# abeytheo/gan-inpainting

Measured on AMD Instinct MI355X. Metric: training images/sec at 256x256 bs=32/GPU, higher is better.
Workload: dtype f16; 1 GPU; wgan_rmse 256x256 bs=32/GPU (BASELINE.json configs[3]): U-Net G (41.8M) + PatchGAN critic, RMSprop 5e-5, clip 0.01, RMSE recon, G update every 5th batch, random-init weights; global_batch=32, parallelism=dp1, compute=fp16 MFMA, fp32 accumulate, fp32 master weights

## Files before the change

### gan-inpainting_amd/backend.py

```python
import ctypes as C
import os
import threading

import torch

_HERE = os.path.dirname(os.path.abspath(__file__))
LIB_PATH = os.environ.get("GI_LIB_PATH") or os.path.join(_HERE, "libganinpaint.so")

GI_F32, GI_F16 = 0, 1
ACT_NONE, ACT_RELU, ACT_LRELU = 0, 1, 2

_vp, _i, _i64, _f, _u64 = C.c_void_p, C.c_int, C.c_int64, C.c_float, C.c_uint64

PROTOTYPES = {
    "gi_last_error": (C.c_char_p, []),
    "gi_version": (_i, []),
    "gi_set_option": (_i, [C.c_char_p, _i]),
    "gi_get_option": (_i, [C.c_char_p, C.POINTER(_i)]),
    "gi_debug_last_kernel": (C.c_char_p, []),
    "gi_debug_fold_count": (_i, []),
    "gi_ctx_create": (_i, [_i, _vp, C.POINTER(_vp)]),
    "gi_ctx_destroy": (_i, [_vp]),
    "gi_ctx_sync": (_i, [_vp]),
    "gi_unet_create": (_i, [_vp, _i, _i, _f, _i, _i, _i, _i, _i, C.POINTER(_vp)]),
    "gi_unet_create_ex": (_i, [_vp, _i, _i, _i, _f, _i, _i, _i, _i, _i, C.POINTER(_vp)]),
    "gi_unet_create_norm": (_i, [_vp, _i, _i, _i, _i, _f, _i, _i, _i, _i, _i, C.POINTER(_vp)]),
    "gi_unet_create_padded": (_i, [_vp, _i, _i, _i, _i, _i, _f, _i, _i, _i, _i, _i, C.POINTER(_vp)]),
    "gi_patchgan_create": (_i, [_vp, _i, _i, _i, _i, _i, _i, C.POINTER(_vp)]),
    "gi_patchgan_create_sn": (_i, [_vp, _i, _i, _i, _i, _i, _i, _i, _i, C.POINTER(_vp)]),
    "gi_net_sn_read": (_i, [_vp, _i, _vp, _vp, _i64]),
    "gi_dcgan_create": (_i, [_vp, _i, _i, _i, _i, _i, C.POINTER(_vp)]),
    "gi_dcgan_debug_forward_convs": (_i, [_vp, _i, _vp, _i]),
    "gi_net_destroy": (_i, [_vp]),
    "gi_net_tensor_count": (_i, [_vp]),
    "gi_net_tensor_desc": (_i, [_vp, _i, C.c_char_p, _i, C.POINTER(_i), C.POINTER(_i64), C.POINTER(_i),
                                C.POINTER(_i64), C.POINTER(_i64)]),
    "gi_net_param_floats": (_i64, [_vp]),
    "gi_net_buffer_floats": (_i64, [_vp]),
    "gi_net_workspace_bytes": (_i64, [_vp]),
    "gi_net_bind": (_i, [_vp, _vp, _vp, _vp, _vp, _i64]),
    "gi_net_sync_weights": (_i, [_vp]),
    "gi_net_set_train": (_i, [_vp, _i]),
    "gi_net_set_inference": (_i, [_vp, _i]),
    "gi_net_set_loss_scale": (_i, [_vp, _f]),
    "gi_net_set_bn_groups": (_i, [_vp, _i]),
    "gi_net_set_dropout_seed": (_i, [_vp, _u64]),
    "gi_net_get_dropout_state": (_i, [_vp, C.POINTER(_u64), C.POINTER(_u64)]),
    "gi_net_set_dropout_state": (_i, [_vp, _u64, _u64]),
    "gi_net_dropout_mask": (_i, [_vp, _i, _i, _vp, _i64]),
    "gi_net_saved_activation": (_i, [_vp, _i, _i, _i, _vp, _i64]),
    "gi_net_debug_nonzero_tickets": (_i, [_vp, _vp]),
    "gi_net_set_dropout_mask": (_i, [_vp, _i, _i, _vp]),
    "gi_net_forward": (_i, [_vp, _i, _vp, _vp, _i]),
    "gi_net_backward": (_i, [_vp, _i, _vp, _vp, _i]),
    "gi_net_backward_phase": (_i, [_vp, _i, _vp, _vp, _i, _i]),
    "gi_net_phase_split": (_i64, [_vp]),
    "gi_net_phase_split2": (_i64, [_vp]),
    "gi_comm_unique_id": (_i, [C.c_char_p]),
    "gi_comm_create": (_i, [C.c_char_p, _i, _i, _i, C.POINTER(_vp)]),
    "gi_comm_destroy": (_i, [_vp]),
    "gi_allreduce_sum_f32": (_i, [_vp, _vp, _i64, _vp]),
    "gi_net_allreduce_grads_async": (_i, [_vp, _vp, _i64, _i64, _vp]),
    "gi_allreduce_wait": (_i, [_vp, _vp, _vp]),
    "gi_patchgan_gradient_penalty": (_i, [_vp, _vp, _i, _f, _vp]),
    "gi_patchgan_gp_saved_activation": (_i, [_vp, _i, _vp, _i64]),
    "gi_interpolate": (_i, [_vp, _vp, _vp, _vp, _i, _i64, _vp]),
    "gi_mask_apply": (_i, [_vp, _vp, _vp, _vp, _vp, _i64, _i]),
    "gi_mask_composite": (_i, [_vp, _vp, _vp, _vp, _vp, _i64]),
    "gi_mul": (_i, [_vp, _vp, _vp, _vp, _i64]),
    "gi_add": (_i, [_vp, _vp, _vp, _vp, _i64, _f]),
    "gi_loss_l1": (_i, [_vp, _vp, _vp, _i64, _vp, _vp, _f, _vp]),
    "gi_loss_rmse": (_i, [_vp, _vp, _vp, _i64, _f, _vp, _vp, _f, _vp]),
    "gi_loss_mse": (_i, [_vp, _vp, _vp, _i64, _vp, _vp, _f, _vp]),
    "gi_loss_local": (_i, [_vp, _vp, _vp, _vp, _i64, _i, _vp, _vp, _f, _vp]),
    "gi_loss_adv": (_i, [_vp, _vp, _i, _i, _f, _vp, _vp, _f]),
    "gi_loss_adv_pair": (_i, [_vp, _vp, _i, _i, _f, _f, _vp, _vp, _vp, _f, _f]),
    "gi_adam_step": (_i, [_vp, _vp, _vp, _vp, _vp, _i64, _f, _f, _f, _f, _i, _f]),
    "gi_rmsprop_step": (_i, [_vp, _vp, _vp, _vp, _i64, _f, _f, _f, _f, _f]),
    "gi_clamp": (_i, [_vp, _vp, _i64, _f, _f]),
    "gi_grad_absmean": (_i, [_vp, _vp, _vp, _vp, _i, _vp]),
    "gi_ssim_scratch_floats": (_i64, [_i, _i, _i, _i, _i]),
    "gi_ssim": (_i, [_vp, _vp, _vp, _i, _i, _i, _i, _i, _vp, _vp, _vp, _vp]),
    "gi_eval_recon_scratch_floats": (_i64, [_i64]),
    "gi_eval_recon": (_i, [_vp, _vp, _vp, _vp, _i64, _f, _vp, _vp, _vp, _vp]),
    "gi_seg_metrics": (_i, [_vp, _vp, _vp, _i, _i, _i64, _vp, _i, _vp, _vp, _vp]),
    "gi_loss_tv": (_i, [_vp, _vp, _i, _i, _i, _f, _vp, _vp, _f, _vp]),
    "gi_loss_cross_entropy": (_i, [_vp, _vp, _vp, _i, _i, _i64, _vp, _i, _vp, _vp, _f, _vp]),
    "gi_vgg19_create": (_i, [_vp, _i, _i, _i, _vp]),
    "gi_vgg19_destroy": (None, [_vp]),
    "gi_vgg19_param_floats": (_i64, [_vp]),
    "gi_vgg19_workspace_bytes": (_i64, [_vp]),
    "gi_vgg19_num_tensors": (_i, [_vp]),
    "gi_vgg19_tensor_desc": (_i, [_vp, _i, _vp, _i, _vp, _vp]),
    "gi_vgg19_bind": (_i, [_vp, _vp, _vp, _i64]),
    "gi_vgg19_sync_weights": (_i, [_vp]),
    "gi_vgg19_perceptual_style": (_i, [_vp, _vp, _vp, _i, _f, _f, _vp, _vp]),
    "gi_vgg19_features": (_i, [_vp, _vp, _i, _i, _vp]),
    "gi_vgg19_grad_workspace_bytes": (_i64, [_vp]),
    "gi_vgg19_bind_grad": (_i, [_vp, _vp, _i64]),
    "gi_vgg19_perceptual_style_grad": (_i, [_vp, _vp, _vp, _i, _f, _f, _vp, _vp, _vp, _f]),
    "gi_vgg19_grad_layer": (_i, [_vp, _i, _vp]),
    "gi_lpips_create": (_i, [_vp, _i, _i, _i, _vp]),
    "gi_lpips_destroy": (None, [_vp]),
# ... 9 lines not shown
    "gi_lpips_bind_grad": (_i, [_vp, _vp, _i64]),
    "gi_lpips_distance_grad": (_i, [_vp, _vp, _vp, _i, _vp, _vp, _vp, _f]),
    "gi_lpips_grad_tap": (_i, [_vp, _i, _vp]),
    "gi_debug_lpips_pack_t": (_i, [_vp, _vp, _vp, _i, _i]),
    "gi_debug_lpips_seed": (_i, [_vp, _i, _vp, _i, _i, _i, _vp, _vp, _vp]),
    "gi_debug_lpips_scale": (_i, [_vp, _vp, _vp, _i]),
    "gi_debug_lpips_act_bwd": (_i, [_vp, _i, _vp, _vp, _vp, _vp, _i, _i, _i, _i, _i]),
    "gi_debug_lpips_conv1_adjoint": (_i, [_vp, _vp, _vp, _vp, _f, _vp, _i, _i, _i]),
    "gi_debug_lpips_conv1": (_i, [_vp, _vp, _vp, _i, _i, _i, _vp, _vp, _vp, _vp]),
    "gi_debug_lpips_fold": (_i, [_vp, _vp, _vp, _vp, _vp, _vp]),
    "gi_debug_lpips_tap_ws_bytes": (_i64, [_i]),
    "gi_debug_lpips_tap": (_i, [_vp, _vp, _i, _i, _i, _i, _vp, _vp, _i64, _vp, _vp]),
    "gi_inception_create": (_i, [_vp, _i, _i, _vp]),
    "gi_inception_destroy": (None, [_vp]),
    "gi_inception_param_floats": (_i64, [_vp]),
    "gi_inception_workspace_bytes": (_i64, [_vp]),
    "gi_inception_num_tensors": (_i, [_vp]),
    "gi_inception_tensor_desc": (_i, [_vp, _i, _vp, _i, _vp, _vp]),
    "gi_inception_bind": (_i, [_vp, _vp, _vp, _i64]),
    "gi_inception_sync_weights": (_i, [_vp]),
    "gi_inception_features": (_i, [_vp, _vp, _i, _i, _i, _i, _vp]),
    "gi_inception_debug_forward_convs": (_i, [_vp, _vp, _i, _i, _i, _i, _i]),
    "gi_inception_num_steps": (_i, [_vp]),
    "gi_inception_step_desc": (_i, [_vp, _i, _vp, _vp, _vp, _vp, _vp]),
    "gi_inception_debug_forward_steps": (_i, [_vp, _vp, _i, _i, _i, _i, _i]),
    "gi_inception_debug_read": (_i, [_vp, _i, _i, _i, _vp]),
    "gi_fid_stats_acc_doubles": (_i64, [_i]),
    "gi_fid_stats_update": (_i, [_vp, _vp, _vp, _i, _i]),
    "gi_fid_stats_finish": (_i, [_vp, _vp, _vp, _vp, _i]),
    "gi_featmetrics_workspace_bytes": (_i64, [_i, _i64, _i64, _i]),
    "gi_kid_subset_sums": (_i, [_vp, _vp, _vp, _vp, _vp, _i, _i, _i, _vp, _i64, _vp]),
    "gi_feat_knn_radius": (_i, [_vp, _vp, _i, _i, _i, _vp, _i64, _vp]),
    "gi_feat_manifold_members": (_i, [_vp, _vp, _i, _vp, _vp, _i, _i, _vp, _i64, _vp, _vp]),
    "gi_debug_feat_gram": (_i, [_vp, _vp, _vp, _i, _vp, _vp, _i, _i, _vp]),
    "gi_resize_output_size": (_i, [_i, _i, _i, _vp, _vp]),
    "gi_resize_table_bytes": (_i64, [_i, _i, _i, _i]),
    "gi_resize_build_tables": (_i, [_vp, _i, _i, _i, _i, _vp]),
    "gi_resize_to_tensor": (_i, [_vp, _vp, _vp, _i, _i, _i, _i, _i, _vp, _vp, _vp]),
    "gi_mask_generate": (_i, [_vp, _i, _u64, _vp, _i, _i, _i, _vp, _vp]),
    "gi_batch_gather": (_i, [_vp, _vp, _i64, _i, _i, _vp, _i, _vp, _u64, _i, _vp]),
    "gi_image_quantize": (_i, [_vp, _vp, _i64, _vp]),
    "gi_panel_assemble": (_i, [_vp, _vp, _i, _i, _i, _i, _i, _vp]),
    "gi_mask_bbox": (_i, [_vp, _vp, _i, _i, _i, _vp]),
    "gi_window_crop": (_i, [_vp, _vp, _i, _i, _i, _i, _i, _i, _i, _vp]),
    "gi_feather_paste": (_i, [_vp, _vp, _vp, _i, _i, _i, _i, _i, _i, _vp, _i, _vp]),
    "gi_mask_components_workspace_bytes": (C.c_size_t, [_i, _i, _i]),
    "gi_mask_components": (_i, [_vp, _vp, _i, _i, _i, _i, _vp, _vp, _vp, _vp]),
    "gi_diffaug_params": (_i, [_vp, _i, _u64, _u64, _i, _i, _i, _vp]),
    "gi_diffaug_fwd": (_i, [_vp, _vp, _vp, _i, _i, _i, _i, _vp]),
    "gi_diffaug_bwd": (_i, [_vp, _vp, _vp, _i, _i, _i, _i, _vp]),
    "gi_diffaug_apply": (_i, [_vp, _i, _u64, _u64, _vp, _i, _i, _i, _vp]),
    "gi_diffaug_apply_bwd": (_i, [_vp, _i, _u64, _u64, _vp, _i, _i, _i, _vp]),
    "gi_check_finite": (_i, [_vp, _vp, _i64, _vp]),
    "gi_check_finite_scan": (_i, [_vp, _vp, _i64, _vp]),
    "gi_check_finite_finish": (_i, [_vp, _vp]),
    "gi_adam_step_guarded": (_i, [_vp, _vp, _vp, _vp, _vp, _i64, _f, _f, _f, _f, _i, _f, _vp]),
    "gi_adam_step_guarded2": (_i, [_vp, _vp, _vp, _vp, _vp, _i64, _f, _f, _f, _f, _i, _i, _f, _vp]),
    "gi_rmsprop_step_guarded": (_i, [_vp, _vp, _vp, _vp, _i64, _f, _f, _f, _f, _f, _vp]),
    "gi_check_finite_scan_word": (_i, [_vp, _vp, _i64, _vp, _i]),
    "gi_adam_step_scan": (_i, [_vp, _vp, _vp, _vp, _vp, _i64, _f, _f, _f, _f, _i, _i, _f, _vp, _i, _i]),
    "gi_rmsprop_step_scan": (_i, [_vp, _vp, _vp, _vp, _i64, _f, _f, _f, _f, _f, _vp, _i, _i]),
    "gi_ema_update": (_i, [_vp, _vp, _vp, _i64, _f, _vp]),
    "gi_wgrad_s2_scratch_bytes": (_i64, [_i, _i, _i, _i, _i, _i]),
    "gi_wgrad_s2_ws": (_i, [_vp, _i, _vp, _vp, _vp, _i, _i, _i, _i, _i, _i, _i, _i, _f, _vp, _i64]),
    "gi_c1_gather": (_i, [_vp, _i, _vp, _vp, _vp, _i, _i, _i, _i, _i, _i, _i, _f, _vp, _vp, _vp]),
    "gi_c1_scatter": (_i, [_vp, _i, _vp, _vp, _vp, _vp, _i, _i, _i, _i, _i, _i, _i, _i, _f, _vp, _vp, _vp, _i, _vp, _vp]),
    "gi_c1_wgrad": (_i, [_vp, _i, _vp, _vp, _vp, _i, _i, _i, _i, _i, _i, _i, _f, _f, _vp, _i, _vp, _vp, _vp, _i64]),
    "gi_c1_wgrad_reduce": (_i, [_vp, _vp, _vp, _i, _i, _vp, _i64]),
    "gi_c1_head4_col_bytes": (_i64, [_i, _i, _i]),
    "gi_c1_head4_forward": (_i, [_vp, _vp, _vp, _vp, _vp, _vp, _i, _i, _i, _i, _i, _i, _vp]),
    "gi_c1_head4_dgrad": (_i, [_vp, _vp, _vp, _vp, _i, _i, _i, _i, _i]),
    "gi_conv_s2_forward": (_i, [_vp, _i, _vp, _vp, _vp, _i, _i, _i, _i, _i, _i, _i, _i, _i, _vp, _i64]),
    "gi_convT_s2_forward": (_i, [_vp, _i, _vp, _vp, _vp, _i, _i, _i, _i, _i, _i, _i, _i, _i, _vp, _i64]),
    "gi_wgrad_s2": (_i, [_vp, _i, _vp, _vp, _vp, _i, _i, _i, _i, _i, _i, _i, _i, _f]),
    "gi_conv_s2_forward_ex": (_i, [_vp, _i, _vp, _vp, _vp, _i, _i, _i, _i, _i, _i, _i, _i, _i, _vp, _i64, _vp]),
    "gi_convT_s2_forward_ex": (_i, [_vp, _i, _vp, _vp, _vp, _i, _i, _i, _i, _i, _i, _i, _i, _i, _vp, _i64, _vp]),
    "gi_debug_igemm_plan": (_i, [_i, _i, _i, _i, _i, _i, _i, _i, _i, _i, _i, _i64, _i, _vp, _i, _vp]),
    "gi_stat_acc_words": (_i64, [_i]),
    "gi_stat_acc_read": (_i, [_vp, _vp, _i, _i, _i, _vp]),
    "gi_debug_col_stats": (_i, [_vp, _i, _vp, _i64, _i, _vp, C.POINTER(_i)]),
    "gi_debug_bn_finalize": (_i, [_vp, _vp, _i, _i, _i64, _vp, _vp, _vp, _vp, _vp, _vp, _vp, _vp, _i, _f, _f, _i, _i64, _i]),
    "gi_debug_bn_apply": (_i, [_vp, _i, _vp, _vp, _i64, _i, _i, _i, _vp, _vp, _i, _vp, _f, _i64, _i]),
    "gi_debug_bn_finalize_acc": (_i, [_vp, _i, _vp]),
    "gi_debug_bn_apply_acc": (_i, [_vp, _i, _vp, _vp, _i64, _i, _i, _i, _i, _vp, _f, _u64, _f, _vp, _vp, _vp, _i64]),
    "gi_debug_act_bn_bwd": (_i, [_vp, _i, _vp]),
    "gi_debug_in_forward": (_i, [_vp, _i, _vp, _vp, _i, _i, _i, _i, _i, _i, _vp, _f, _f, _vp]),
    "gi_debug_act_in_bwd": (_i, [_vp, _i, _vp, _i, _i, _vp]),
    "gi_debug_bias_grad": (_i, [_vp, _i, _vp, _i64, _i, _f, _vp, _vp]),
    "gi_debug_tanh_bwd": (_i, [_vp, _vp, _vp, _vp, _i64, _f]),
    "gi_debug_fill_dropout": (_i, [_vp, _vp, _i64, _u64, _f]),
    "gi_debug_mask_layout": (_i, [_vp, _vp, _vp, _i, _i, _i, _i]),
    "gi_debug_mul_slope": (_i, [_vp, _i, _vp, _vp, _vp, _i64]),
    "gi_debug_bn_tangent_inject": (_i, [_vp, _i, _vp, _vp, _vp, _vp, _vp, _i64, _i, _vp, _vp, _vp, _vp, _f, _vp, _vp]),
    "gi_debug_gp_direction": (_i, [_vp, _vp, _i, _i64, _f, _vp, _vp, _vp, _vp, _vp]),
    "gi_debug_gp_unscale_add": (_i, [_vp, _vp, _vp, _vp, _i64]),
    "gi_debug_sn_power_iteration": (_i, [_vp, _vp, _i, _i, _i, _vp, _vp, _i, _i, _vp]),
    "gi_debug_sn_project_add": (_i, [_vp, _vp, _vp, _vp, _vp, _vp, _i, _i, _i, _vp, _vp]),
    "gi_debug_stat_acc_add": (_i, [_vp, _vp, _i, _i, _i, _i, _vp, _i]),
    "gi_debug_pack_weights_batch": (_i, [_vp, _i, _vp, _i]),
    "gi_debug_head_forward": (_i, [_vp, _i, _vp]),
    "gi_debug_head_backward": (_i, [_vp, _i, _vp]),
    "gi_debug_head_scratch_bytes": (_i64, [_i, _i, _i]),
    "gi_debug_vgg_conv3x3": (_i, [_vp, _vp, _vp, _vp, _vp, _i, _i, _i, _i, _i, _i, _vp, _i, _i, _vp, _vp, C.POINTER(_i), C.POINTER(_i)]),
    "gi_debug_vgg_conv1": (_i, [_vp, _vp, _vp, _i, _i, _i, _vp, _vp, _vp, _vp]),
    "gi_debug_vgg_maxpool2": (_i, [_vp, _vp, _vp, _i, _i, _i, _i]),
    "gi_debug_vgg_tap_ws_bytes": (_i64, []),
    "gi_debug_vgg_tap_terms": (_i, [_vp, _vp, _i, _i, _i, _i, _vp, _i64, _vp, _vp, _vp, C.POINTER(_i)]),
    "gi_debug_vgg_seed": (_i, [_vp, _i, _vp, _vp, _vp, _vp, _vp, _vp, _i, _i, _i, _f, _f]),
    "gi_debug_vgg_scale": (_i, [_vp, _vp, _vp]),
    "gi_debug_vgg_act_bwd": (_i, [_vp, _i, _vp, _vp, _vp, _vp, _i, _i, _i, _i, _i]),
    "gi_debug_vgg_conv1_adjoint": (_i, [_vp, _vp, _vp, _vp, _f, _vp, _i, _i, _i]),
    "gi_pack_weights": (_i, [_vp, _i, _vp, _i, _i, _vp, _vp]),
    "gi_convert": (_i, [_vp, _i, _vp, _vp, _i64]),
    "gi_convert_back": (_i, [_vp, _i, _vp, _vp, _i64]),
    "gi_time_convT_s2": (_i, [_vp, _i, _vp, _vp, _vp, _i, _i, _i, _i, _i, _i, _i, _i, C.POINTER(_f)]),
    "gi_time_conv_s2": (_i, [_vp, _i, _vp, _vp, _vp, _i, _i, _i, _i, _i, _i, _i, _i, C.POINTER(_f)]),
}

_lib = None
_lock = threading.Lock()


class IgemmEx(C.Structure):
    _fields_ = [("relu_cend", _i),
                ("mask", _vp), ("ldmask", _i), ("mask_slope", _f),
                ("add", _vp), ("ldadd", _i),
                ("mask_bits", _vp),
                ("stat_acc", _vp), ("stat_reps", _i), ("stat_pg", _i),
                ("partials", _vp),
                ("bwd_x", _vp), ("bwd_ldx", _i),
                ("bwd_scale", _vp), ("bwd_shift", _vp), ("bwd_mean", _vp), ("bwd_inv", _vp), ("bwd_stride", _i),
                ("bwd_slope", _f), ("bwd_acc", _vp), ("bwd_reps", _i), ("bwd_pg", _i64),
                ("bwd_c0", _i), ("bwd_c", _i),
                ("mask_applied", _i), ("bwd_applied", _i), ("stat_used", _i), ("ntiles_out", _i)]


class BnAccArgs(C.Structure):
    _fields_ = [("acc", _vp), ("reps", _i),
                ("gamma", _vp), ("beta", _vp), ("running_mean", _vp), ("running_var", _vp),
                ("scale", _vp), ("shift", _vp), ("save_mean", _vp), ("save_invstd", _vp),
                ("count", _i64), ("momentum", _f), ("eps", _f), ("groups", _i), ("out_stride", _i),
                ("zero_next", _vp), ("zero_words", _i)]


class ActBnBwdArgs(C.Structure):
    _fields_ = [("g1", _vp), ("ldg1", _i), ("coffg1", _i),
                ("g2", _vp), ("ldg2", _i), ("coffg2", _i),
                ("y", _vp), ("ldy", _i), ("coffy", _i),
                ("x", _vp), ("dx", _vp),
                ("pixels", _i64), ("c", _i), ("act", _i), ("drop_scale", _f),
                ("has_bn", _i), ("eval_bn", _i),
                ("gamma", _vp), ("save_mean", _vp), ("save_invstd", _vp),
                ("dgamma", _vp), ("dbeta", _vp), ("inv_loss_scale", _f),
                ("partials", _vp), ("sums", _vp), ("fwd_scale", _vp), ("fwd_shift", _vp),
                ("groups", _i), ("stat_stride", _i),
                ("acc", _vp), ("acc_reps", _i), ("zero_next", _vp), ("zero_words", _i),
                ("reduce_done", _i)]


class PackJob(C.Structure):
    _fields_ = [("w", _vp), ("packed", _vp), ("phase", _vp),
                ("ca", _i), ("cb", _i), ("scale_on_b", _i),
                ("scale", _vp)]


class HeadArgs(C.Structure):
# ... 98 lines not shown
```

### gan-inpainting_amd/csrc/api.hip

```cpp
#include <string.h>

#include <stdlib.h>

#include "common.h"
#include "stat_acc.h"
#include "igemm_plan.h"

static thread_local char g_err[1024] = "";

void gi_set_error(const char* fmt, ...) {
  va_list ap;
  va_start(ap, fmt);
  vsnprintf(g_err, sizeof(g_err), fmt, ap);
  va_end(ap);
}

namespace {
struct OptDesc { const char* name; int dflt; int value; int state; };
inline int opt_load(const int& v) { return __atomic_load_n(&v, __ATOMIC_RELAXED); }
inline void opt_store(int& v, int x) { __atomic_store_n(&v, x, __ATOMIC_RELAXED); }
OptDesc g_opts[GI_OPT_COUNT] = {
  {"GI_IGEMM5", 7, 0, 0}, {"GI_IGEMM6", 1, 0, 0}, {"GI_IGEMM7", 1, 0, 0}, {"GI_IGEMM_FIXUP", 1, 0, 0}, {"GI_IGEMM_VARIANT", 3, 0, 0},
  {"GI_BN_ACC", 1, 0, 0}, {"GI_FUSE_HEAD", 1, 0, 0}, {"GI_HEAD_FAST", 1, 0, 0}, {"GI_BN_BWD_FUSE", 1, 0, 0}, {"GI_BN_BWD_SMALL", 512, 0, 0},
  {"GI_WGRAD2", 1, 0, 0}, {"GI_WGRAD3", 1, 0, 0}, {"GI_IGEMM8", 1, 0, 0}, {"GI_BN_FOLD", 0, 0, 0}, {"GI_C1_FUSED", 1, 0, 0},
  {"GI_WGRAD_STREAM", 1, 0, 0}, {"GI_MASK_BITS", 1, 0, 0}, {"GI_C1W_FUSE", 1, 0, 0}, {"GI_IGEMM7_WAVES", 8, 0, 0},
};
thread_local const char* g_last_kernel = "";
int g_fold_count = 0;
}
void gi_note_fold() { __atomic_fetch_add(&g_fold_count, 1, __ATOMIC_RELAXED); }

int gi_opt(int id) {
  OptDesc& o = g_opts[id];
  if (opt_load(o.state) == 0) {
    const char* e = getenv(o.name);
    opt_store(o.value, e ? atoi(e) : o.dflt);
    __atomic_store_n(&o.state, 1, __ATOMIC_RELEASE);
  }
  return opt_load(o.value);
}
void gi_note_kernel(const char* name) { g_last_kernel = name; }

extern "C" {

int gi_set_option(const char* name, int value) {
  GI_REQUIRE(name, "set_option: null name");
  for (int i = 0; i < GI_OPT_COUNT; ++i)
    if (strcmp(name, g_opts[i].name) == 0) {
      if (value < 0) opt_store(g_opts[i].state, 0);
      else { opt_store(g_opts[i].value, value); __atomic_store_n(&g_opts[i].state, 2, __ATOMIC_RELEASE); }
      return GI_OK;
    }
  gi_set_error("set_option: unknown option '%s'", name);
  return GI_ERR_INVALID;
}
int gi_get_option(const char* name, int* value) {
  GI_REQUIRE(name && value, "get_option: null argument");
  for (int i = 0; i < GI_OPT_COUNT; ++i)
    if (strcmp(name, g_opts[i].name) == 0) { *value = gi_opt(i); return GI_OK; }
  gi_set_error("get_option: unknown option '%s'", name);
  return GI_ERR_INVALID;
}
const char* gi_debug_last_kernel(void) { return g_last_kernel; }
int gi_debug_fold_count(void) { return __atomic_load_n(&g_fold_count, __ATOMIC_RELAXED); }

const char* gi_last_error(void) { return g_err; }
int gi_version(void) { return 100; }

int gi_ctx_create(int device_id, void* hip_stream, gi_ctx** out) {
  GI_REQUIRE(out != nullptr, "ctx_create: out is null");
  int count = 0;
  GI_HIP(hipGetDeviceCount(&count));
  GI_REQUIRE(device_id >= 0 && device_id < count, "ctx_create: device %d not present (%d visible)", device_id, count);
  GI_HIP(hipSetDevice(device_id));
  hipDeviceProp_t prop;
  GI_HIP(hipGetDeviceProperties(&prop, device_id));
  if (strncmp(prop.gcnArchName, "gfx950", 6) != 0) {
    gi_set_error("ctx_create: device %d is %s; this library is built for gfx950 only", device_id, prop.gcnArchName);
    return GI_ERR_UNSUPPORTED;
  }
  gi_ctx* c = new gi_ctx();
  c->device = device_id;
  c->stream = (hipStream_t)hip_stream;
  *out = c;
  return GI_OK;
}
int gi_ctx_destroy(gi_ctx* ctx) {
  if (ctx && ctx->tickets) (void)hipFree(ctx->tickets);
  if (ctx && ctx->absmean_partials) (void)hipFree(ctx->absmean_partials);
  if (ctx && ctx->diffaug_partials) (void)hipFree(ctx->diffaug_partials);
  delete ctx;
  return GI_OK;
}
int gi_ctx_sync(gi_ctx* ctx) {
  GI_REQUIRE(ctx, "ctx_sync: null");
  GI_HIP(hipStreamSynchronize(ctx->stream));
  return GI_OK;
}

static unsigned* ctx_tickets(gi_ctx* ctx) {
  if (!ctx->tickets) {
    if (hipMalloc((void**)&ctx->tickets, GI_IGEMM_TICKETS * 4) != hipSuccess) { ctx->tickets = nullptr; return nullptr; }
    if (hipMemset(ctx->tickets, 0, GI_IGEMM_TICKETS * 4) != hipSuccess) { (void)hipFree(ctx->tickets); ctx->tickets = nullptr; }
  }
  return ctx->tickets;
}

int gi_conv_s2_forward(gi_ctx* ctx, int dtype, const void* in, const void* w_packed, void* out, int n, int H, int W, int cb, int ldin,
                       int ca, int ldout, int relu_in, int act_out, float* ws, int64_t ws_bytes) {
  GI_REQUIRE(ctx && in && w_packed && out, "conv_s2_forward: null pointer");
  GI_REQUIRE(H % 2 == 0 && W % 2 == 0, "conv_s2_forward: H=%d W=%d must be even", H, W);
  IgemmArgs a;
  memset(&a, 0, sizeof(a));
  a.in = in; a.w = w_packed; a.out = out; a.ws = ws; a.ws_bytes = ws_bytes;
  a.tickets = ws ? ctx_tickets(ctx) : nullptr;
  a.n = n; a.Hs = H / 2; a.Ws = W / 2;
  a.cin = cb; a.ldin = ldin; a.cout = ca; a.ldout = ldout;
  a.relu_in = relu_in; a.act_out = act_out;
  return op_igemm(ctx->stream, dtype, 0, a);
}

int gi_convT_s2_forward(gi_ctx* ctx, int dtype, const void* in, const void* w_phase, void* out, int n, int H, int W, int ca, int ldin,
                        int cb, int ldout, int relu_in, int act_out, float* ws, int64_t ws_bytes) {
  GI_REQUIRE(ctx && in && w_phase && out, "convT_s2_forward: null pointer");
  IgemmArgs a;
  memset(&a, 0, sizeof(a));
  a.in = in; a.w = w_phase; a.out = out; a.ws = ws; a.ws_bytes = ws_bytes;
  a.tickets = ws ? ctx_tickets(ctx) : nullptr;
  a.n = n; a.Hs = H; a.Ws = W;
  a.cin = ca; a.ldin = ldin; a.cout = cb; a.ldout = ldout;
  a.relu_in = relu_in; a.act_out = act_out;
  return op_igemm(ctx->stream, dtype, 1, a);
}

static int apply_ex(IgemmArgs& a, const gi_igemm_ex* ex) {
  if (!ex) return GI_OK;
  GI_REQUIRE(ex->relu_cend >= 0 && ex->relu_cend % 64 == 0 && ex->relu_cend <= a.cin, "igemm_ex: relu_cend=%d must be a multiple of 64 within the %d input channels",
             ex->relu_cend, a.cin);
  a.relu_cend = ex->relu_cend;
  a.mask = ex->mask; a.ldmask = ex->ldmask; a.mask_slope = ex->mask_slope;
  a.add = ex->add; a.ldadd = ex->ldadd;
  a.mask_bits = ex->mask ? ex->mask_bits : nullptr;
  a.stat_acc = ex->stat_acc; a.stat_reps = ex->stat_reps; a.stat_pg = ex->stat_pg;
  a.partials = ex->partials;
  a.bwd_x = ex->bwd_x; a.bwd_ldx = ex->bwd_ldx; a.bwd_scale = ex->bwd_scale; a.bwd_shift = ex->bwd_shift; a.bwd_mean = ex->bwd_mean;
  a.bwd_inv = ex->bwd_inv; a.bwd_stride = ex->bwd_stride; a.bwd_slope = ex->bwd_slope; a.bwd_acc = ex->bwd_acc; a.bwd_reps = ex->bwd_reps;
  a.bwd_pg = ex->bwd_pg;
  a.bwd_c0 = ex->bwd_c0; a.bwd_c = ex->bwd_c;
  return GI_OK;
}
static void return_ex(const IgemmArgs& a, gi_igemm_ex* ex) {
  if (!ex) return;
  ex->mask_applied = a.mask_applied; ex->bwd_applied = a.bwd_applied; ex->stat_used = a.stat_used; ex->ntiles_out = a.ntiles_out;
}

int gi_conv_s2_forward_ex(gi_ctx* ctx, int dtype, const void* in, const void* w_packed, void* out, int n, int H, int W, int cb, int ldin,
                          int ca, int ldout, int relu_in, int act_out, float* ws, int64_t ws_bytes, gi_igemm_ex* ex) {
  GI_REQUIRE(ctx && in && w_packed && out, "conv_s2_forward_ex: null pointer");
  GI_REQUIRE(H % 2 == 0 && W % 2 == 0, "conv_s2_forward_ex: H=%d W=%d must be even", H, W);
  IgemmArgs a;
  memset(&a, 0, sizeof(a));
  a.in = in; a.w = w_packed; a.out = out; a.ws = ws; a.ws_bytes = ws_bytes;
  a.tickets = ws ? ctx_tickets(ctx) : nullptr;
  a.n = n; a.Hs = H / 2; a.Ws = W / 2;
  a.cin = cb; a.ldin = ldin; a.cout = ca; a.ldout = ldout;
  a.relu_in = relu_in; a.act_out = act_out;
  GI_TRY(apply_ex(a, ex));
  const int rc = op_igemm(ctx->stream, dtype, 0, a);
  return_ex(a, ex);
  return rc;
}

int gi_convT_s2_forward_ex(gi_ctx* ctx, int dtype, const void* in, const void* w_phase, void* out, int n, int H, int W, int ca, int ldin,
                           int cb, int ldout, int relu_in, int act_out, float* ws, int64_t ws_bytes, gi_igemm_ex* ex) {
  GI_REQUIRE(ctx && in && w_phase && out, "convT_s2_forward_ex: null pointer");
  IgemmArgs a;
  memset(&a, 0, sizeof(a));
  a.in = in; a.w = w_phase; a.out = out; a.ws = ws; a.ws_bytes = ws_bytes;
  a.tickets = ws ? ctx_tickets(ctx) : nullptr;
  a.n = n; a.Hs = H; a.Ws = W;
  a.cin = ca; a.ldin = ldin; a.cout = cb; a.ldout = ldout;
  a.relu_in = relu_in; a.act_out = act_out;
  GI_TRY(apply_ex(a, ex));
  const int rc = op_igemm(ctx->stream, dtype, 1, a);
  return_ex(a, ex);
  return rc;
}

int gi_debug_igemm_plan(int dtype, int mode, int n, int Hs, int Ws, int cin, int ldin, int cout, int ldout, int relu_in, int act_out,
                        int64_t ws_bytes, int has_tickets, const gi_igemm_ex* ex, int offered, gi_igemm_plan_info* out) {
  GI_REQUIRE(out, "debug_igemm_plan: null pointer");
  static char dummy[8];
  IgemmArgs a;
  memset(&a, 0, sizeof(a));
  a.in = a.w = a.out = dummy;
  if (ws_bytes > 0) { a.ws = (float*)dummy; a.ws_bytes = ws_bytes; }
  a.tickets = has_tickets ? (unsigned*)dummy : nullptr;
  a.n = n; a.Hs = Hs; a.Ws = Ws;
  a.cin = cin; a.ldin = ldin; a.cout = cout; a.ldout = ldout;
  a.relu_in = relu_in; a.act_out = act_out;
  GI_TRY(apply_ex(a, ex));
  IgemmFold fold = {};
  if ((offered & 1) && a.stat_acc) { fold.bn.groups = 1; fold.bn.acc = a.stat_acc; fold.lddst = ldout; fold.act = GI_ACT_RELU; a.fold = &fold; }
  if ((offered & 2) && a.mask_bits) { a.c1w_img = (const float*)dummy; a.c1w_part = (float*)dummy; a.c1w_part_floats = (int64_t)1 << 40; a.c1w_scale = 1.f; }
  if (offered & 4) a.pool2 = 1;
  if (offered & 8) a.bias = (const float*)dummy;
  IgemmPlan p;
  GI_TRY(gi_igemm_plan(dtype, mode, a, &p));
  gi_igemm_returns(p, a);
  memset(out, 0, sizeof(*out));
  strncpy(out->name, p.name, sizeof(out->name) - 1);
  out->grid = p.grid; out->splitk = p.splitk > 1 ? p.splitk : 1; out->ntiles_out = a.ntiles_out;
  out->mask_applied = a.mask_applied; out->bwd_applied = a.bwd_applied; out->stat_used = a.stat_used;
  out->c1w_applied = a.c1w_applied; out->c1w_blocks = a.c1w_blocks; out->pool_applied = a.pool_applied; out->fold_applied = a.fold_applied;
  return GI_OK;
}

int64_t gi_stat_acc_words(int c) { return gi_stat_block_words(c, GI_STAT_MAXREP); }

namespace {
__global__ void __launch_bounds__(256) stat_acc_read_kernel(const unsigned long long* acc, int c, int reps, int group, double* out) {
  for (int ch = blockIdx.x * 256 + threadIdx.x; ch < c; ch += gridDim.x * 256) {
    out[ch] = gi_stat_read(acc, c, reps, group, 0, ch);
    out[c + ch] = gi_stat_read(acc, c, reps, group, 1, ch);
  }
}
}

int gi_stat_acc_read(gi_ctx* ctx, const unsigned long long* acc, int c, int reps, int group, double* out_dev) {
  GI_REQUIRE(ctx && acc && out_dev && c > 0 && reps >= 1 && reps <= GI_STAT_MAXREP && (group == 0 || group == 1), "stat_acc_read: bad argument");
  hipLaunchKernelGGL(stat_acc_read_kernel, dim3((c + 255) / 256), dim3(256), 0, ctx->stream, acc, c, reps, group, out_dev);
  GI_LAUNCH_CHECK();
  return GI_OK;
}

int gi_wgrad_s2(gi_ctx* ctx, int dtype, const void* S, const void* L, float* dW, int n, int Hs, int Ws, int ca, int ldS, int cb, int ldL,
                int relu_S, float scale) {
  GI_REQUIRE(ctx && S && L && dW, "wgrad_s2: null pointer");
  WgradArgs a;
  a.S = S; a.L = L; a.dW = dW; a.n = n; a.Hs = Hs; a.Ws = Ws;
  a.ca = ca; a.ldS = ldS; a.coffS = 0; a.cb = cb; a.ldL = ldL; a.coffL = 0;
  a.relu_S = relu_S; a.scale = scale;
  a.scratch = nullptr; a.scratch_bytes = 0;
  return op_wgrad(ctx->stream, dtype, a);
}

int64_t gi_wgrad_s2_scratch_bytes(int dtype, int n, int Hs, int Ws, int ca, int cb) {
  return op_wgrad_scratch_bytes(dtype, n, Hs, Ws, ca, cb);
}

int gi_wgrad_s2_ws(gi_ctx* ctx, int dtype, const void* S, const void* L, float* dW, int n, int Hs, int Ws, int ca, int ldS, int cb, int ldL,
                   int relu_S, float scale, float* scratch, int64_t scratch_bytes) {
  GI_REQUIRE(ctx && S && L && dW, "wgrad_s2_ws: null pointer");
  WgradArgs a;
  a.S = S; a.L = L; a.dW = dW; a.n = n; a.Hs = Hs; a.Ws = Ws;
  a.ca = ca; a.ldS = ldS; a.coffS = 0; a.cb = cb; a.ldL = ldL; a.coffL = 0;
  a.relu_S = relu_S; a.scale = scale;
  a.scratch = scratch; a.scratch_bytes = scratch_bytes;
  return op_wgrad(ctx->stream, dtype, a);
}


int gi_c1_gather(gi_ctx* ctx, int dtype, const float* img, const float* w, void* out, int n, int Hs, int Ws, int c, int ldout, int coffout,
                 int act_out, float in_scale, const float* bias, unsigned long long* bits, int* bits_written) {
  GI_REQUIRE(ctx && img && w && out, "c1_gather: null pointer");
  return op_c1_gather(ctx->stream, dtype, img, w, out, n, Hs, Ws, c, ldout, coffout, act_out, in_scale, bias, bits, bits_written);
}

int gi_c1_scatter(gi_ctx* ctx, int dtype, const void* X, const float* w, const float* bias, float* img, int n, int Hs, int Ws, int c, int ldx,
                  int coffx, int relu_in, int post, float out_scale, void* col_scratch, float* img2, const void* x2, int ld2,
                  const float* scale2, const float* shift2) {
  GI_REQUIRE(ctx && X && w && img, "c1_scatter: null pointer");
  GI_REQUIRE(!x2 || (scale2 && shift2), "c1_scatter: x2 without scale2 / shift2");
  C1Affine aff;
  aff.x2 = x2; aff.ld2 = ld2; aff.scale = scale2; aff.shift = shift2;
  return op_c1_scatter(ctx->stream, dtype, X, w, bias, img, n, Hs, Ws, c, ldx, coffx, relu_in, post, out_scale, col_scratch, img2,
                       x2 ? &aff : nullptr);
}

int gi_c1_wgrad(gi_ctx* ctx, int dtype, const void* X, const float* img, float* dW, int n, int Hs, int Ws, int c, int ldx, int coffx,
                int relu_in, float scale, float img_scale, const void* x2, int ld2, const float* scale2, const float* shift2, float* scratch,
                int64_t scratch_floats) {
  GI_REQUIRE(ctx && X && img && dW, "c1_wgrad: null pointer");
  GI_REQUIRE(!x2 || (scale2 && shift2), "c1_wgrad: x2 without scale2 / shift2");
  C1Affine aff;
  aff.x2 = x2; aff.ld2 = ld2; aff.scale = scale2; aff.shift = shift2;
  return op_c1_wgrad(ctx->stream, dtype, X, img, dW, n, Hs, Ws, c, ldx, coffx, relu_in, scale, img_scale, x2 ? &aff : nullptr, scratch,
                     scratch_floats);
}
// ... 23 lines not shown
inline bool dbg_act_ok(int act) { return act == GI_ACT_NONE || act == GI_ACT_RELU || act == GI_ACT_LRELU; }
inline bool dbg_c_ok(int dtype, int c) { const int e = dbg_epc(dtype); return c > 0 && c % e == 0 && gi_is_pow2(c / e) && c / e <= 256; }
inline bool dbg_view_ok(int dtype, int c, int ld, int coff) { const int e = dbg_epc(dtype); return coff >= 0 && coff % e == 0 && ld % e == 0 && coff + c <= ld; }

int dbg_bn_acc(const char* who, int c, const gi_bn_acc_args* b, BnAccArgs& o) {
  GI_REQUIRE(b && b->acc && b->gamma && b->beta && b->running_mean && b->running_var && b->scale && b->shift && b->save_mean && b->save_invstd,
             "%s: null pointer", who);
  GI_REQUIRE(b->reps >= 1 && b->reps <= GI_STAT_MAXREP, "%s: reps=%d outside 1..%d", who, b->reps, GI_STAT_MAXREP);
  GI_REQUIRE(b->groups == 1 || b->groups == 2, "%s: groups=%d (1 or 2)", who, b->groups);
  GI_REQUIRE(b->count >= 1, "%s: count=%lld", who, (long long)b->count);
  GI_REQUIRE(b->groups == 1 || b->out_stride >= c, "%s: out_stride=%d below the %d channels", who, b->out_stride, c);
  GI_REQUIRE(b->zero_words >= 0 && (b->zero_words == 0 || b->zero_next), "%s: zero_words=%d without zero_next", who, b->zero_words);
  o.acc = b->acc; o.reps = b->reps; o.gamma = b->gamma; o.beta = b->beta; o.running_mean = b->running_mean; o.running_var = b->running_var;
  o.scale = b->scale; o.shift = b->shift; o.save_mean = b->save_mean; o.save_invstd = b->save_invstd;
  o.count = b->count; o.momentum = b->momentum; o.eps = b->eps; o.groups = b->groups; o.out_stride = b->out_stride;
  o.zero_next = b->zero_words > 0 ? b->zero_next : nullptr; o.zero_words = b->zero_words;
  return GI_OK;
}

int dbg_bwd_args(const char* who, int dtype, const gi_act_bn_bwd_args* s, bool chunks_pow2, ActBnBwdArgs& a) {
  GI_REQUIRE(s && s->dx, "%s: null pointer", who);
  GI_REQUIRE(dbg_dtype_ok(dtype) && dbg_act_ok(s->act), "%s: dtype=%d act=%d", who, dtype, s->act);
  GI_REQUIRE(chunks_pow2 ? dbg_c_ok(dtype, s->c) : (s->c > 0 && s->c % dbg_epc(dtype) == 0), "%s: c=%d unsupported", who, s->c);
  GI_REQUIRE(s->pixels >= 1, "%s: pixels=%lld", who, (long long)s->pixels);
  GI_REQUIRE(s->g1 || s->g2, "%s: no upstream gradient", who);
  GI_REQUIRE(!s->g1 || dbg_view_ok(dtype, s->c, s->ldg1, s->coffg1), "%s: g1 ld=%d coff=%d for %d channels", who, s->ldg1, s->coffg1, s->c);
  GI_REQUIRE(!s->g2 || dbg_view_ok(dtype, s->c, s->ldg2, s->coffg2), "%s: g2 ld=%d coff=%d for %d channels", who, s->ldg2, s->coffg2, s->c);
  GI_REQUIRE(!s->y || dbg_view_ok(dtype, s->c, s->ldy, s->coffy), "%s: y ld=%d coff=%d for %d channels", who, s->ldy, s->coffy, s->c);
  GI_REQUIRE(s->drop_scale == 1.f || s->act == GI_ACT_RELU,
             "%s: drop_scale=%g with act=%d: the backward takes the dropout zeros from y > 0, which only a ReLU output can carry", who,
             (double)s->drop_scale, s->act);
  memset(&a, 0, sizeof(a));
  a.g1 = s->g1; a.ldg1 = s->ldg1; a.coffg1 = s->coffg1;
  a.g2 = s->g2; a.ldg2 = s->ldg2; a.coffg2 = s->coffg2;
  a.y = s->y; a.ldy = s->ldy; a.coffy = s->coffy;
  a.x = s->x; a.dx = s->dx; a.pixels = s->pixels; a.c = s->c; a.act = s->act; a.drop_scale = s->drop_scale;
  a.has_bn = s->has_bn; a.eval_bn = s->eval_bn;
  a.gamma = s->gamma; a.save_mean = s->save_mean; a.save_invstd = s->save_invstd;
  a.dgamma = s->dgamma; a.dbeta = s->dbeta; a.inv_loss_scale = s->inv_loss_scale;
  a.partials = s->partials; a.sums = s->sums; a.fwd_scale = s->fwd_scale; a.fwd_shift = s->fwd_shift;
  a.groups = s->groups; a.stat_stride = s->stat_stride;
  a.acc = s->acc; a.acc_reps = s->acc_reps; a.zero_next = s->zero_words > 0 ? s->zero_next : nullptr; a.zero_words = s->zero_words;
  a.reduce_done = s->reduce_done;
  return GI_OK;
}

__global__ void __launch_bounds__(256) stat_acc_add_kernel(unsigned long long* acc, int c, int reps, int group, int q, const float* addends) {
  const int r = blockIdx.x;
  for (int ch = threadIdx.x; ch < c; ch += 256) gi_stat_add(acc, c, r & (reps - 1), group, q, ch, addends[(int64_t)r * c + ch]);
}
}

int gi_debug_col_stats(gi_ctx* ctx, int dtype, const void* x, int64_t pixels, int c, float* partials, int* rows_out) {
  GI_REQUIRE(ctx && x && partials && rows_out, "debug_col_stats: null pointer");
  GI_REQUIRE(dbg_dtype_ok(dtype) && pixels >= 1, "debug_col_stats: dtype=%d pixels=%lld", dtype, (long long)pixels);
  return op_col_stats(ctx->stream, dtype, x, pixels, c, partials, rows_out);
}

int gi_debug_bn_finalize(gi_ctx* ctx, const float* partials, int rows, int c, int64_t count, const float* gamma, const float* beta,
                         float* running_mean, float* running_var, float* scale, float* shift, float* save_mean, float* save_invstd, int train,
                         float momentum, float eps, int groups, int64_t part_stride, int out_stride) {
  GI_REQUIRE(ctx && gamma && beta && running_mean && running_var && scale && shift && save_mean && save_invstd, "debug_bn_finalize: null pointer");
  GI_REQUIRE(!train || (partials && rows >= 1), "debug_bn_finalize: train mode needs partial rows (rows=%d)", rows);
  GI_REQUIRE(c >= 1 && count >= 1, "debug_bn_finalize: c=%d count=%lld", c, (long long)count);
  GI_REQUIRE(groups == 1 || groups == 2, "debug_bn_finalize: groups=%d (1 or 2)", groups);
  GI_REQUIRE(groups == 1 || (out_stride >= c && (!train || part_stride >= (int64_t)rows * 2 * c)),
             "debug_bn_finalize: two populations overlap (part_stride=%lld out_stride=%d)", (long long)part_stride, out_stride);
  return op_bn_finalize(ctx->stream, partials, rows, c, count, gamma, beta, running_mean, running_var, scale, shift, save_mean, save_invstd, train,
                        momentum, eps, groups, part_stride, out_stride);
}

int gi_debug_bn_apply(gi_ctx* ctx, int dtype, const void* x, void* y, int64_t pixels, int c, int ldy, int coffy, const float* scale,
                      const float* shift, int act, const uint8_t* drop_mask, float drop_scale, int64_t pg, int gstride) {
  GI_REQUIRE(ctx && x && y, "debug_bn_apply: null pointer");
  GI_REQUIRE(dbg_dtype_ok(dtype) && dbg_act_ok(act) && pixels >= 1, "debug_bn_apply: dtype=%d act=%d pixels=%lld", dtype, act, (long long)pixels);
  GI_REQUIRE(dbg_c_ok(dtype, c), "debug_bn_apply: c=%d unsupported", c);
  GI_REQUIRE(dbg_view_ok(dtype, c, ldy, coffy), "debug_bn_apply: ldy=%d coffy=%d for %d channels", ldy, coffy, c);
  GI_REQUIRE((scale == nullptr) == (shift == nullptr), "debug_bn_apply: scale and shift go together");
  GI_REQUIRE(pg >= 0 && pg <= pixels, "debug_bn_apply: pg=%lld of %lld pixels", (long long)pg, (long long)pixels);
  GI_REQUIRE(!(pg > 0 && pg < pixels) || gstride >= c, "debug_bn_apply: gstride=%d below the %d channels", gstride, c);
  return op_bn_apply(ctx->stream, dtype, x, y, pixels, c, ldy, coffy, scale, shift, act, drop_mask, drop_scale, pg, gstride);
}

int gi_debug_bn_finalize_acc(gi_ctx* ctx, int c, const gi_bn_acc_args* b) {
  GI_REQUIRE(ctx && c >= 1, "debug_bn_finalize_acc: bad argument");
  BnAccArgs o;
  GI_TRY(dbg_bn_acc("debug_bn_finalize_acc", c, b, o));
  return op_bn_finalize_acc(ctx->stream, c, o);
}

int gi_debug_bn_apply_acc(gi_ctx* ctx, int dtype, const void* x, void* y, int64_t pixels, int c, int ldy, int coffy, int act, uint8_t* drop_mask,
                          float drop_scale, uint64_t drop_seed, float drop_p, const gi_bn_acc_args* b, const void* side_src, void* side_dst,
                          int64_t side_bytes) {
  GI_REQUIRE(ctx && x && y, "debug_bn_apply_acc: null pointer");
  GI_REQUIRE(dbg_dtype_ok(dtype) && dbg_act_ok(act) && pixels >= 1, "debug_bn_apply_acc: dtype=%d act=%d pixels=%lld", dtype, act, (long long)pixels);
  GI_REQUIRE(dbg_c_ok(dtype, c), "debug_bn_apply_acc: c=%d unsupported", c);
  GI_REQUIRE(dbg_view_ok(dtype, c, ldy, coffy), "debug_bn_apply_acc: ldy=%d coffy=%d for %d channels", ldy, coffy, c);
  GI_REQUIRE(drop_p >= 0.f && drop_p < 1.f && (drop_p == 0.f || drop_mask), "debug_bn_apply_acc: drop_p=%g needs a mask to store the draw", (double)drop_p);
  GI_REQUIRE(side_bytes >= 0, "debug_bn_apply_acc: side_bytes=%lld", (long long)side_bytes);
  BnAccArgs o;
  GI_TRY(dbg_bn_acc("debug_bn_apply_acc", c, b, o));
  return op_bn_apply_acc(ctx->stream, dtype, x, y, pixels, c, ldy, coffy, act, drop_mask, drop_scale, drop_seed, drop_p, o, side_src, side_dst,
                         side_bytes);
}

int gi_debug_act_bn_bwd(gi_ctx* ctx, int dtype, const gi_act_bn_bwd_args* s) {
  GI_REQUIRE(ctx, "debug_act_bn_bwd: null context");
  ActBnBwdArgs a;
  GI_TRY(dbg_bwd_args("debug_act_bn_bwd", dtype, s, true, a));
  GI_REQUIRE(a.groups == 1 || a.groups == 2, "debug_act_bn_bwd: groups=%d (1 or 2)", a.groups);
  GI_REQUIRE(a.groups == 1 || a.stat_stride >= a.c, "debug_act_bn_bwd: stat_stride=%d below the %d channels", a.stat_stride, a.c);
  GI_REQUIRE(!a.has_bn || (a.x && a.gamma && a.save_mean && a.save_invstd), "debug_act_bn_bwd: BatchNorm without x / gamma / save_mean / save_invstd");
  GI_REQUIRE((a.fwd_scale == nullptr) == (a.fwd_shift == nullptr), "debug_act_bn_bwd: fwd_scale and fwd_shift go together");
  const bool need_y = a.g2 != nullptr || a.act != GI_ACT_NONE;
  GI_REQUIRE(!need_y || a.y || (a.has_bn && a.fwd_scale), "debug_act_bn_bwd: the activation's sign needs y or fwd_scale / fwd_shift");
  GI_REQUIRE(!a.acc || (a.acc_reps >= 1 && a.acc_reps <= GI_STAT_MAXREP), "debug_act_bn_bwd: acc_reps=%d outside 1..%d", a.acc_reps, GI_STAT_MAXREP);
  GI_REQUIRE(!a.reduce_done || (a.acc && a.has_bn && !a.eval_bn), "debug_act_bn_bwd: reduce_done needs train-mode accumulators");
  GI_REQUIRE(!a.has_bn || a.acc || (a.partials && a.sums), "debug_act_bn_bwd: BatchNorm without accumulators needs partials and sums");
  GI_REQUIRE(a.zero_words >= 0, "debug_act_bn_bwd: zero_words=%d", a.zero_words);
  return op_act_bn_bwd(ctx->stream, dtype, a);
}

int gi_debug_in_forward(gi_ctx* ctx, int dtype, const void* x, void* y, int n, int hw, int c, int ldy, int coffy, int act,
                        const uint8_t* drop_mask, float drop_scale, float eps, float* stats) {
  GI_REQUIRE(ctx && x && y && stats, "debug_in_forward: null pointer");
  GI_REQUIRE(dbg_dtype_ok(dtype) && dbg_act_ok(act), "debug_in_forward: dtype=%d act=%d", dtype, act);
  GI_REQUIRE(c > 0 && c % dbg_epc(dtype) == 0 && dbg_view_ok(dtype, c, ldy, coffy), "debug_in_forward: c=%d ldy=%d coffy=%d", c, ldy, coffy);
  return op_in_forward(ctx->stream, dtype, x, y, n, hw, c, ldy, coffy, act, drop_mask, drop_scale, eps, stats);
}

int gi_debug_act_in_bwd(gi_ctx* ctx, int dtype, const gi_act_bn_bwd_args* s, int n, int hw, const float* stats) {
  GI_REQUIRE(ctx && stats, "debug_act_in_bwd: null pointer");
  ActBnBwdArgs a;
  GI_TRY(dbg_bwd_args("debug_act_in_bwd", dtype, s, false, a));
  GI_REQUIRE(n >= 1 && hw >= 1, "debug_act_in_bwd: n=%d hw=%d", n, hw);
  const bool need_y = a.g2 != nullptr || a.act != GI_ACT_NONE;
  GI_REQUIRE(!need_y || a.y, "debug_act_in_bwd: the activation's sign needs y");
  return op_act_in_bwd(ctx->stream, dtype, a, n, hw, stats);
}

int gi_debug_bias_grad(gi_ctx* ctx, int dtype, const void* dz, int64_t pixels, int c, float scale, float* dbias, float* partials) {
  GI_REQUIRE(ctx && dz && dbias && partials, "debug_bias_grad: null pointer");
  GI_REQUIRE(dbg_dtype_ok(dtype) && pixels >= 1, "debug_bias_grad: dtype=%d pixels=%lld", dtype, (long long)pixels);
  return op_bias_grad(ctx->stream, dtype, dz, pixels, c, scale, dbias, partials);
}

int gi_debug_tanh_bwd(gi_ctx* ctx, const float* dy, const float* y, float* dx, int64_t count, float scale) {
  GI_REQUIRE(ctx && dy && y && dx && count >= 0, "debug_tanh_bwd: bad argument");
  return op_tanh_bwd(ctx->stream, dy, y, dx, count, scale);
}

int gi_debug_fill_dropout(gi_ctx* ctx, uint8_t* mask_nhwc, int64_t count, uint64_t seed, float p) {
  GI_REQUIRE(ctx && mask_nhwc && count >= 0, "debug_fill_dropout: bad argument");
  GI_REQUIRE(p >= 0.f && p < 1.f, "debug_fill_dropout: p=%g outside [0, 1)", (double)p);
  return op_fill_dropout(ctx->stream, mask_nhwc, count, seed, p);
}

int gi_debug_mask_layout(gi_ctx* ctx, const uint8_t* src, uint8_t* dst, int n, int c, int hw, int to_nhwc) {
  GI_REQUIRE(ctx && src && dst && src != dst, "debug_mask_layout: bad pointer");
  GI_REQUIRE(n >= 1 && c >= 1 && hw >= 1, "debug_mask_layout: n=%d c=%d hw=%d", n, c, hw);
  return op_mask_nchw_to_nhwc(ctx->stream, src, dst, n, c, hw, to_nhwc);
}

int gi_debug_mul_slope(gi_ctx* ctx, int dtype, const void* tin, const void* a, void* tout, int64_t count) {
  GI_REQUIRE(ctx && tin && a && tout, "debug_mul_slope: null pointer");
  GI_REQUIRE(dbg_dtype_ok(dtype) && count >= 0, "debug_mul_slope: dtype=%d count=%lld", dtype, (long long)count);
// ... 178 lines not shown
```

### gan-inpainting_amd/csrc/bn_acc.h

```cpp
#pragma once
#include "common.h"
#include "stat_acc.h"

struct BnAccP {
  const unsigned long long* acc;
  int reps;
  const float* gamma; const float* beta;
  float* rmean; float* rvar;
  float* scale; float* shift; float* smean; float* sinv;
  double count;
  float momentum, eps;
  int groups, out_stride;
  unsigned long long* zero_next;
  int zero_words;
};
static inline void gi_fill_acc_params(BnAccP& fa, const BnAccArgs& b) {
  fa.acc = b.acc; fa.reps = b.reps > 0 ? b.reps : 1; fa.gamma = b.gamma; fa.beta = b.beta; fa.rmean = b.running_mean; fa.rvar = b.running_var;
  fa.scale = b.scale; fa.shift = b.shift; fa.smean = b.save_mean; fa.sinv = b.save_invstd;
  fa.count = (double)b.count; fa.momentum = b.momentum; fa.eps = b.eps; fa.groups = b.groups; fa.out_stride = b.out_stride;
  fa.zero_next = b.zero_next; fa.zero_words = b.zero_words;
}
__device__ __forceinline__ void zero_words64(unsigned long long* p, int n) {
  for (int i = threadIdx.x; i < n; i += 256) p[i] = 0ull;
}
template <bool COHERENT = false>
__device__ __forceinline__ void bn_from_acc(const BnAccP& a, int c, int ch, int j, bool write, float& sc_out, float& sh_out) {
  const float gam = a.gamma[ch], bet = a.beta[ch];
  float rm = 0.f, rv = 0.f;
  if (write) { rm = a.rmean[ch]; rv = a.rvar[ch]; }
  double t0, t1;
  gi_stat_read2<COHERENT>(a.acc, c, a.reps, j, ch, t0, t1);
  const double m = t0 / a.count;
  double v = t1 / a.count - m * m;
  if (v < 0.0 || a.count <= 1.0) v = 0.0;
  const float mean = (float)m, var = (float)v;
  const float inv = 1.0f / sqrtf(var + a.eps);
  const float sc = gam * inv;
  sc_out = sc;
  sh_out = bet - mean * sc;
  if (write) {
    const float unbiased = a.count > 1.0 ? (float)(v * a.count / (a.count - 1.0)) : var;
    a.rmean[ch] = (1.f - a.momentum) * rm + a.momentum * mean;
    a.rvar[ch] = (1.f - a.momentum) * rv + a.momentum * unbiased;
    const int o = j * a.out_stride + ch;
    a.scale[o] = sc;
    a.shift[o] = sh_out;
    a.smean[o] = mean;
    a.sinv[o] = inv;
  }
}

__host__ __device__ __forceinline__ uint64_t gi_mix64(uint64_t z) {
  z = (z ^ (z >> 30)) * 0xBF58476D1CE4E5B9ull;
  z = (z ^ (z >> 27)) * 0x94D049BB133111EBull;
  return z ^ (z >> 31);
}
constexpr uint64_t GI_GOLDEN64 = 0x9E3779B97F4A7C15ull;
__device__ __forceinline__ uint8_t dropout_keep(uint64_t seed, int64_t i, uint32_t thresh) {
  const uint64_t z = gi_mix64(seed + GI_GOLDEN64 * (uint64_t)(i + 1));
  return ((uint32_t)(z >> 32) >= thresh) ? 1 : 0;
}
static inline uint32_t gi_dropout_thresh(float p) {
  const double t = (double)p * 4294967296.0;
  const uint32_t thresh = t >= 4294967295.0 ? 0xFFFFFFFFu : (uint32_t)t;
  return thresh ? thresh : 1u;
}
```

### gan-inpainting_amd/csrc/common.h

```cpp
#pragma once
#include <hip/hip_runtime.h>
#include <stdint.h>
#include <stdio.h>
#include <stdarg.h>
#include <mutex>
#include <type_traits>

#include "../../include/ganinpaint.h"

typedef _Float16 half_t;
typedef _Float16 h8_t __attribute__((ext_vector_type(8)));
typedef _Float16 h4_t __attribute__((ext_vector_type(4)));
typedef _Float16 h2_t __attribute__((ext_vector_type(2)));
typedef __fp16 fp16x4_t __attribute__((__vector_size__(4 * sizeof(__fp16))));
typedef float f4_t __attribute__((ext_vector_type(4)));
typedef unsigned int u4_t __attribute__((ext_vector_type(4)));
typedef float f16_t __attribute__((ext_vector_type(16)));

void gi_set_error(const char* fmt, ...);

enum gi_opt_id {
  GI_OPT_IGEMM5 = 0, GI_OPT_IGEMM6, GI_OPT_IGEMM7, GI_OPT_IGEMM_FIXUP, GI_OPT_IGEMM_VARIANT, GI_OPT_BN_ACC, GI_OPT_FUSE_HEAD,
  GI_OPT_HEAD_FAST, GI_OPT_BN_BWD_FUSE, GI_OPT_BN_BWD_SMALL, GI_OPT_WGRAD2, GI_OPT_WGRAD3, GI_OPT_IGEMM8, GI_OPT_BN_FOLD, GI_OPT_C1_FUSED, GI_OPT_WGRAD_STREAM, GI_OPT_MASK_BITS, GI_OPT_C1W_FUSE, GI_OPT_IGEMM7_WAVES, GI_OPT_COUNT
};
int gi_opt(int id);
void gi_note_kernel(const char* name);
void gi_note_fold();
#ifdef GI_ABLATION
#include <stdlib.h>
static inline int gi_tune(const char* env, int dflt) { const char* e = getenv(env); return e ? atoi(e) : dflt; }
#else
#define gi_tune(env, dflt) (dflt)
#endif

template <int N, typename F>
__host__ __device__ __forceinline__ void static_for(F&& f) {
  if constexpr (N > 0) {
    static_for<N - 1>(f);
    f(std::integral_constant<int, N - 1>{});
  }
}

template <int ACT>
__device__ __forceinline__ float gi_act_c(float v) {
  if constexpr (ACT == GI_ACT_RELU) return v > 0.f ? v : 0.f;
  else if constexpr (ACT == GI_ACT_LRELU) return v > 0.f ? v : 0.2f * v;
  else return v;
}
template <typename F>
__device__ __forceinline__ void gi_with_act(int act, F&& f) {
  if (act == GI_ACT_NONE) f(std::integral_constant<int, GI_ACT_NONE>{});
  else if (act == GI_ACT_RELU) f(std::integral_constant<int, GI_ACT_RELU>{});
  else f(std::integral_constant<int, GI_ACT_LRELU>{});
}
template <typename F>
__host__ __device__ __forceinline__ void gi_with_bool(bool b, F&& f) {
  if (b) f(std::true_type{});
  else f(std::false_type{});
}
template <int CTRL>
__device__ __forceinline__ float gi_dpp(float v) {
  return __builtin_bit_cast(float, __builtin_amdgcn_update_dpp(0, __builtin_bit_cast(int, v), CTRL, 0xF, 0xF, true));
}
__device__ __forceinline__ float gi_row16_sum(float v) {
  v += gi_dpp<0xB1>(v);
  v += gi_dpp<0x4E>(v);
  v += gi_dpp<0x141>(v);
  v += gi_dpp<0x140>(v);
  return v;
}

__device__ __forceinline__ f4_t gi_ordered_sum_f4(const f4_t* part, int64_t stride, int k0, int k1, f4_t s) {
  int k = k0;
  for (; k + 8 <= k1; k += 8) {
    f4_t v[8];
#pragma unroll
    for (int j = 0; j < 8; ++j) v[j] = part[(int64_t)(k + j) * stride];
#pragma unroll
    for (int j = 0; j < 8; ++j) s += v[j];
  }
  if (k + 4 <= k1) {
    f4_t v[4];
#pragma unroll
    for (int j = 0; j < 4; ++j) v[j] = part[(int64_t)(k + j) * stride];
#pragma unroll
    for (int j = 0; j < 4; ++j) s += v[j];
    k += 4;
  }
  if (k + 2 <= k1) {
    const f4_t v0 = part[(int64_t)k * stride], v1 = part[(int64_t)(k + 1) * stride];
    s += v0;
    s += v1;
    k += 2;
  }
  if (k < k1) s += part[(int64_t)k * stride];
  return s;
}

struct GiDevOnce {
  unsigned long long mask = 0;
  std::mutex mu;
  bool first() {
    int d = 0;
    (void)hipGetDevice(&d);
    const unsigned long long b = 1ull << (d & 63);
    const unsigned long long old = __atomic_fetch_or(&mask, b, __ATOMIC_RELAXED);
    return (old & b) == 0;
  }
  template <typename F>
  hipError_t once(F&& f) {
    int d = 0;
    (void)hipGetDevice(&d);
    const unsigned long long b = 1ull << (d & 63);
    if (__atomic_load_n(&mask, __ATOMIC_ACQUIRE) & b) return hipSuccess;
    std::lock_guard<std::mutex> lock(mu);
    if (__atomic_load_n(&mask, __ATOMIC_RELAXED) & b) return hipSuccess;
    const hipError_t e = f();
    if (e == hipSuccess) __atomic_fetch_or(&mask, b, __ATOMIC_RELEASE);
    return e;
  }
};

#define GI_HIP(expr)                                                                  \
// ... 14 lines not shown
    }                                                                                 \
  } while (0)

#define GI_REQUIRE(cond, ...)                                                         \
  do {                                                                                \
    if (!(cond)) {                                                                    \
      gi_set_error(__VA_ARGS__);                                                      \
      return GI_ERR_INVALID;                                                          \
    }                                                                                 \
  } while (0)

#define GI_TRY(expr)                \
  do {                              \
    int _s = (expr);                \
    if (_s != GI_OK) return _s;     \
  } while (0)

template <auto Kernel, typename P>
int gi_launch_lds(dim3 grid, int block, int lds, int lds_attr, hipStream_t st, const P& p) {
  static GiDevOnce attr_set;
  GI_HIP(attr_set.once([&] { return hipFuncSetAttribute((const void*)Kernel, hipFuncAttributeMaxDynamicSharedMemorySize, lds_attr); }));
  hipLaunchKernelGGL(Kernel, grid, dim3(block), lds, st, p);
  GI_LAUNCH_CHECK();
  return GI_OK;
}

struct gi_ctx {
  int device;
  hipStream_t stream;
  unsigned* tickets = nullptr;
  double* absmean_partials = nullptr;
  double* diffaug_partials = nullptr;
};

static inline size_t gi_dtype_size(int dtype) { return dtype == GI_F16 ? 2 : 4; }
static inline int64_t gi_align_up(int64_t v, int64_t a) { return (v + a - 1) / a * a; }
static inline int gi_ilog2(int v) {
  int l = 0;
  while ((1 << l) < v) ++l;
  return l;
}
static inline bool gi_is_pow2(int v) { return v > 0 && (v & (v - 1)) == 0; }
static inline int grid_for(int64_t work_items, int per_block, int cap) {
  int64_t b = (work_items + per_block - 1) / per_block;
  if (b > cap) b = cap;
  if (b < 1) b = 1;
  return (int)b;
}


struct IgemmFold;
struct IgemmArgs {
  const void* in;
  const void* w;
  void* out;
  const float* bias;
  float* partials;
  float* ws;
  int64_t ws_bytes;
  int n, Hs, Ws;
  int cin, ldin, coffin;
  int cout, ldout, coffout;
  int relu_in;
  int relu_cend;
  int act_out;
  int force_splitk;
  unsigned* tickets;
  int ntiles_out;
  const void* mask; int ldmask, coffmask; float mask_slope;
  const void* add; int ldadd, coffadd;
  int mask_applied;
  const unsigned long long* mask_bits;
  const float* c1w_img; float* c1w_part; int64_t c1w_part_floats; float c1w_scale; int c1w_skip_out;
  int c1w_applied, c1w_blocks;
  unsigned long long* stat_acc; int stat_pg; int stat_reps;
  const void* bwd_x; int bwd_ldx;
  const float* bwd_scale; const float* bwd_shift; const float* bwd_mean; const float* bwd_inv; int bwd_stride;
  float bwd_slope; int bwd_c0, bwd_c;
  unsigned long long* bwd_acc; int bwd_reps; int64_t bwd_pg;
  int bwd_applied;
  int pool2, pool_applied;
  int stat_used;
  const IgemmFold* fold; int fold_applied;
};
constexpr int GI_IGEMM_TICKETS = 1024;
int op_igemm(hipStream_t st, int dtype, int mode, IgemmArgs& a);

struct WgradArgs {
  const void* S;
  const void* L;
  float* dW;
  int n, Hs, Ws;
  int ca, ldS, coffS;
  int cb, ldL, coffL;
  int relu_S;
  float scale;
  float* scratch;
  int64_t scratch_bytes;
};
int op_wgrad(hipStream_t st, int dtype, const WgradArgs& a);
int64_t op_wgrad_scratch_bytes(int dtype, int n, int Hs, int Ws, int ca, int cb);

int op_c1_gather(hipStream_t st, int dtype, const float* img, const float* w, void* out, int n, int Hs,
                 int Ws, int c, int ldout, int coffout, int act_out, float in_scale, const float* bias = nullptr,
                 unsigned long long* bits = nullptr, int* bits_written = nullptr);
struct BnAccArgs;
struct C1Affine { const void* x2; int ld2; const float* scale; const float* shift;
                  const BnAccArgs* bn = nullptr; };
bool op_c1_head4_ok(int dtype, int c, int out_c, int Ws, int ldx, int coffx);
int64_t op_c1_head4_col_bytes(int n, int Hs, int Ws);
int op_c1_head4_forward(hipStream_t st, const void* X, const float* w, const float* bias, float* out, float* out2, int n, int Hs, int Ws, int ldx,
                        int coffx, int relu_in, void* col_scratch);
int op_c1_head4_dgrad(hipStream_t st, const float* g, const float* w, void* out, int n, int Hs, int Ws, int ldout, int coffout);
int op_c1_wgrad_reduce(hipStream_t st, const float* part, float* dW, int count, int blocks, float* scratch = nullptr, int64_t scratch_floats = 0);
bool op_c1_affine_ok(int dtype, int c, int Ws, int ldx, int coffx);
int op_c1_scatter(hipStream_t st, int dtype, const void* X, const float* w, const float* bias, float* img,
                  int n, int Hs, int Ws, int c, int ldx, int coffx, int relu_in, int post, float out_scale,
                  void* col_scratch, float* img2 = nullptr, const C1Affine* aff = nullptr);
int op_c1_wgrad(hipStream_t st, int dtype, const void* X, const float* img, float* dW, int n, int Hs, int Ws,
                int c, int ldx, int coffx, int relu_in, float scale, float img_scale, const C1Affine* aff = nullptr,
                float* scratch = nullptr, int64_t scratch_floats = 0);

int op_bn_finalize(hipStream_t st, const float* partials, int rows, int c, int64_t count, const float* gamma,
                   const float* beta, float* running_mean, float* running_var, float* scale, float* shift,
                   float* save_mean, float* save_invstd, int train, float momentum, float eps, int groups = 1,
                   int64_t part_stride = 0, int out_stride = 0);
struct BnAccArgs {
  const unsigned long long* acc; int reps;
  const float* gamma; const float* beta;
  float* running_mean; float* running_var;
  float* scale; float* shift; float* save_mean; float* save_invstd;
  int64_t count;
  float momentum, eps;
  int groups, out_stride;
  unsigned long long* zero_next; int zero_words;
};
int op_bn_finalize_acc(hipStream_t st, int c, const BnAccArgs& b);
struct IgemmFold {
  BnAccArgs bn;
  void* dst; int lddst, coffdst;
  int act;
  uint8_t* drop_mask; float drop_scale; uint64_t drop_seed; float drop_p;
};
int op_bn_apply_acc(hipStream_t st, int dtype, const void* x, void* y, int64_t pixels, int c, int ldy, int coffy, int act,
                    uint8_t* drop_mask, float drop_scale, uint64_t drop_seed, float drop_p, const BnAccArgs& b,
                    const void* side_src = nullptr, void* side_dst = nullptr, int64_t side_bytes = 0);
int op_bn_apply(hipStream_t st, int dtype, const void* x, void* y, int64_t pixels, int c, int ldy, int coffy,
                const float* scale, const float* shift, int act, const uint8_t* drop_mask, float drop_scale,
                int64_t pg = 0, int gstride = 0);
int op_col_stats(hipStream_t st, int dtype, const void* x, int64_t pixels, int c, float* partials, int* rows_out);

struct ActBnBwdArgs {
  const void* g1; int ldg1, coffg1;
  const void* g2; int ldg2, coffg2;
  const void* y;  int ldy, coffy;
  const void* x;
  void* dx;
  int64_t pixels; int c;
  int act; float drop_scale;
  int has_bn;
  int eval_bn;
  const float* gamma; const float* save_mean; const float* save_invstd;
  float* dgamma; float* dbeta;
  float inv_loss_scale;
  float* partials;
  float* sums;
// ... 98 lines not shown
```

### gan-inpainting_amd/csrc/igemm7.hip

```cpp
#include <stdlib.h>

#include "common.h"
#include "stat_acc.h"
#include "bn_acc.h"
#include "igemm_plan.h"

namespace {

struct KP7 {
  const char* in;
  const char* w;
  char* out;
  const char* zero;
  const float* bias;
  float* partials;
  unsigned long long* stat_acc; int stat_pg, stat_reps;
  float* ws;
  unsigned* tickets;
  int M, Hs, Ws;
  int cin, ldin, coffin;
  int cout, ldout, coffout;
  int Ktot, nk, splitk, kt_per_split;
  int relu_in, act_out, relu_cend;
  int Hin, Win, Hout, Wout;
  int mtiles, ntiles;
  int dbg;
  int fold;
  unsigned* col_tickets;
  BnAccP fa;
  char* fdst; int flddst, fcoffdst, fact;
  uint8_t* fdrop; float fdrop_scale; uint64_t fdrop_seed; uint32_t fdrop_thresh;
};

__device__ __forceinline__ h8_t relu7(h8_t v, short floor) {
  typedef short s8_t __attribute__((ext_vector_type(8)));
  s8_t h = __builtin_bit_cast(s8_t, v);
  const s8_t z = {floor, floor, floor, floor, floor, floor, floor, floor};
  h = __builtin_elementwise_max(h, z);
  return __builtin_bit_cast(h8_t, h);
}
__device__ __forceinline__ void glds16_7(const char* src, char* lds_wave_base) {
  __builtin_amdgcn_global_load_lds((const __attribute__((address_space(1))) void*)src, (__attribute__((address_space(3))) void*)lds_wave_base,
                                   16, 0, 0);
}
template <int N>
__device__ __forceinline__ void wait_vm7() {
  static_assert(N >= 0 && N <= 63, "unexpected DMA count");
  if constexpr (N == 0) asm volatile("s_waitcnt vmcnt(0)" ::: "memory");
  else if constexpr (N == 3) asm volatile("s_waitcnt vmcnt(3)" ::: "memory");
  else if constexpr (N == 4) asm volatile("s_waitcnt vmcnt(4)" ::: "memory");
  else if constexpr (N == 6) asm volatile("s_waitcnt vmcnt(6)" ::: "memory");
  else if constexpr (N == 8) asm volatile("s_waitcnt vmcnt(8)" ::: "memory");
  else if constexpr (N == 12) asm volatile("s_waitcnt vmcnt(12)" ::: "memory");
  else if constexpr (N == 16) asm volatile("s_waitcnt vmcnt(16)" ::: "memory");
  else if constexpr (N == 18) asm volatile("s_waitcnt vmcnt(18)" ::: "memory");
  else if constexpr (N == 24) asm volatile("s_waitcnt vmcnt(24)" ::: "memory");
  else if constexpr (N == 32) asm volatile("s_waitcnt vmcnt(32)" ::: "memory");
  else static_assert(N < 0, "add the immediate");
}

template <int PHASE, int BN, int NSTG_, int PF_, int NW>
__global__ void __launch_bounds__(NW * 64, NW == 4 ? 2 : 1) igemm7_kernel(KP7 p) {
  static_assert(NW == 4 || NW == 8, "four or eight waves");
  constexpr int BM = 128, BK = 64, NTHR = NW * 64;
  constexpr int NWM = (NW == 8 && BN == 64) ? 4 : 2, NWN = NW / NWM;
  constexpr int A_BYTES = BM * 128, B_BYTES = BN * 128, STAGE = A_BYTES + B_BYTES;
  constexpr int NSTG = NSTG_;
  constexpr int AH = NSTG - 1;
  constexpr int AJ = (BM / 8) / NW, BJ = (BN / 8) / NW;
  constexpr int NPC = AJ + BJ;
  constexpr int WM = BM / NWM, WN = BN / NWN, MT = WM / 16, NT = WN / 16;
  static_assert(MT >= 1 && NT >= 1 && MT * NT >= 4, "wave tile");
  extern __shared__ __attribute__((aligned(16))) char smem[];
  __shared__ int s_last;

  const int tid = threadIdx.x, lane = tid & 63;
  const int wave = __builtin_amdgcn_readfirstlane(tid >> 6);
  const int wm = wave / NWN, wn = wave % NWN;

  const int nph = PHASE == 1 ? 4 : 1;
  const int nyz = p.ntiles * nph * p.splitk;
  const int bid = blockIdx.x;
  int mt_idx, yz;
  if (p.mtiles >= 8) {
    const int xcd = bid & 7, local = bid >> 3;
    mt_idx = (local / nyz) * 8 + xcd;
    yz = local % nyz;
    if (mt_idx >= p.mtiles) return;
  } else {
    mt_idx = bid % p.mtiles;
    yz = bid / p.mtiles;
  }
  const int ks = yz % p.splitk;
  const int t2 = yz / p.splitk;
  const int nt_idx = t2 % p.ntiles;
  const int ph = t2 / p.ntiles;
  const int py = ph >> 1, px = ph & 1;
  const int m0 = mt_idx * BM, n0 = nt_idx * BN;
  const char* wptr = p.w + (PHASE == 1 ? (int64_t)ph * p.cout * p.Ktot * 2 : 0);
  const int kt0 = ks * p.kt_per_split;
  const int kt1 = min(p.nk, kt0 + p.kt_per_split);
#ifdef GI_ABLATION
  const int nk = (p.dbg & 8) ? 1 : kt1 - kt0;
#else
  const int nk = kt1 - kt0;
#endif

  const int lrow = lane >> 3;
  const int lchunk = (lane & 7) ^ (lrow & 7);
  int abase[AJ];
  unsigned amask[AJ];
#pragma unroll
  for (int j = 0; j < AJ; ++j) {
    const int m = m0 + (wave * AJ + j) * 8 + lrow;
    abase[j] = 0;
    amask[j] = 0;
    if (m < p.M) {
      const int x = m % p.Ws;
      const int t = m / p.Ws;
      const int y = t % p.Hs;
      const int n = t / p.Hs;
      if (PHASE) {
        const int y0 = y + py, x0 = x + px;
// ... 415 lines not shown
```

### gan-inpainting_amd/csrc/igemm_plan.h

```cpp
#pragma once
#include "common.h"

enum { GI_FAM_GENERIC = 0, GI_FAM_IGEMM3, GI_FAM_IGEMM5, GI_FAM_IGEMM6, GI_FAM_IGEMM7, GI_FAM_IGEMM8 };

struct IgemmPlan {
  int family;
  int variant;
  int mode, bn;
  bool dual, relu;
  int nw, nstg, pf;
  int BM; bool half_n;
  int splitk, kt_per_split;
  bool fixup, finish_launch, atomics_ws;
  bool fold, take_mask, take_mask_bits, take_c1w, take_bwd, bwd_range, take_pool, stat_to_acc;
  int TH, TW, mtiles, ntiles, grid, lds_bytes, lds_attr_bytes, ntiles_out;
  int finish_rows, finish_blocks;
  const char* name;
};
int gi_igemm_plan(int dtype, int mode, const IgemmArgs& a, IgemmPlan* p);

void gi_igemm_returns(const IgemmPlan& p, IgemmArgs& a);

int launch_igemm(hipStream_t st, int dtype, const IgemmPlan& p, const IgemmArgs& a);
int launch_igemm3(hipStream_t st, const IgemmPlan& p, const IgemmArgs& a);
int launch_igemm5(hipStream_t st, const IgemmPlan& p, const IgemmArgs& a);
int launch_igemm7(hipStream_t st, const IgemmPlan& p, const IgemmArgs& a);
int launch_igemm8(hipStream_t st, const IgemmPlan& p, const IgemmArgs& a);
const char* gi_igemm3_zero_page(int dev);
static inline const char* gi_igemm_zero_page() { int dev = 0; return hipGetDevice(&dev) == hipSuccess ? gi_igemm3_zero_page(dev) : nullptr; }

#define GI_IGEMM3_KERNELS(X)  \
  X(0, 0, 128, "igemm3<0,128>") X(1, 1, 128, "igemm3<1,128>") X(2, 2, 128, "igemm3<2,128>") \
  X(3, 0, 64, "igemm3<0,64>") X(4, 1, 64, "igemm3<1,64>") X(5, 2, 64, "igemm3<2,64>")
#define GI_IGEMM5_KERNELS(X)  \
  X(0, 0, 128, "igemm5<0,128>") X(1, 1, 128, "igemm5<1,128>") X(2, 2, 128, "igemm5<2,128>") \
  X(3, 0, 64, "igemm5<0,64>") X(4, 1, 64, "igemm5<1,64>") X(5, 2, 64, "igemm5<2,64>")
#define GI_IGEMM5_DUAL_KERNEL(X) X(6, 3, 128, "igemm5<3,128>")
#define GI_IGEMM6_KERNELS(X)  \
  X(0, 0, 128, false, "igemm6<0,128>") X(2, 1, 128, false, "igemm6<1,128>") X(3, 1, 128, true, "igemm6<1,128,relu>") \
  X(4, 0, 64, false, "igemm6<0,64>") X(6, 1, 64, false, "igemm6<1,64>") X(7, 1, 64, true, "igemm6<1,64,relu>") \
  X(8, 3, 128, false, "igemm6<3,128>") X(9, 3, 128, true, "igemm6<3,128,relu>")
#define GI_IGEMM7_KERNELS(X)  \
  X(0, 0, 128, "igemm7<0,128>") X(1, 1, 128, "igemm7<1,128>") X(2, 0, 64, "igemm7<0,64>") X(3, 1, 64, "igemm7<1,64>")
#define GI_IGEMM7_FOLD_NAMES(X) X(4, 0, 128, "igemm7<0,128>+bn") X(5, 1, 128, "igemm7<1,128>+bn") X(6, 0, 64, "igemm7<0,64>+bn") X(7, 1, 64, "igemm7<1,64>+bn")
#define GI_IGEMM8_KERNELS(X)  \
  X(7, 2, false, 64, "igemm8<2,64>") X(0, 0, false, 128, "igemm8<0>") X(1, 0, true, 128, "igemm8<0,relu>") X(2, 1, false, 128, "igemm8<1>") \
  X(3, 1, true, 128, "igemm8<1,relu>") X(4, 3, false, 128, "igemm8<3>") X(5, 3, true, 128, "igemm8<3,relu>") X(6, 2, false, 128, "igemm8<2>")
```

### gan-inpainting_amd/csrc/igemm_plan.hip

```cpp
#include "igemm_plan.h"

namespace {

constexpr int NEXT = 1;

#define GI_NAME3(V, A, B, NAME) case V: return NAME;
#define GI_NAME4(V, A, B, C, NAME) case V: return NAME;
#define GI_NAME_FN(FN, ROWS) const char* FN(int variant) { switch (variant) { ROWS } return ""; }
GI_NAME_FN(name3, GI_IGEMM3_KERNELS(GI_NAME3))
GI_NAME_FN(name5, GI_IGEMM5_KERNELS(GI_NAME3) GI_IGEMM5_DUAL_KERNEL(GI_NAME3))
GI_NAME_FN(name6, GI_IGEMM6_KERNELS(GI_NAME4))
GI_NAME_FN(name7, GI_IGEMM7_KERNELS(GI_NAME3) GI_IGEMM7_FOLD_NAMES(GI_NAME3))
GI_NAME_FN(name8, GI_IGEMM8_KERNELS(GI_NAME4))

int plan_halo(int mode, const IgemmArgs& a, IgemmPlan& p) {
  if (!gi_is_pow2(a.Ws) || a.Ws < 8) return NEXT;
  const int TW = a.Ws < 32 ? a.Ws : 32, TH = 256 / TW;
  if (a.Hs % TH != 0) return NEXT;
  if (mode == 2 ? (TH + 2) * (TW + 2) > 384 : (TH + 1) * (TW + ((mode == 1 && a.cout % 128 != 0) ? 2 : 1)) > 320) return NEXT;
  int BN = (a.cout % 128 == 0) ? 128 : 64;
  const int nph = mode == 1 ? 4 : 1;
  const int mtiles = a.n * (a.Ws / TW) * (a.Hs / TH);
  if (mode != 2 && mtiles * (a.cout / BN) * nph < 128) return NEXT;
  if (mode == 0 && BN == 128 && mtiles * (a.cout / BN) < 256) {
    if (gi_tune("GI_IGEMM5_NARROW", 1)) BN = 64;
  }
  const bool dual = mode == 1 && BN == 64;
  const int64_t in_px = (int64_t)a.n * a.Hs * a.Ws * (mode == 0 ? 4 : 1), out_px = (int64_t)a.n * a.Hs * a.Ws * (mode == 1 ? 4 : 1);
  GI_REQUIRE(in_px * a.ldin < (1ll << 31) && out_px * a.ldout < (1ll << 31), "igemm5: tensor too large for 32-bit offsets");
  GI_REQUIRE(!a.stat_acc || a.stat_pg == 0 || a.stat_pg % (a.Hs * a.Ws) == 0, "igemm5: stat_pg=%d must be whole images", a.stat_pg);
  if (a.mask) {
    GI_REQUIRE(a.ldmask % 8 == 0 && a.coffmask % 8 == 0 && out_px * a.ldmask < (1ll << 31), "igemm5: mask layout");
    GI_REQUIRE(!a.add || (a.ldadd % 8 == 0 && a.coffadd % 8 == 0 && out_px * a.ldadd < (1ll << 31)), "igemm5: add layout");
  }
  p.take_mask = a.mask != nullptr;
  p.mode = dual ? 3 : mode; p.bn = BN; p.dual = dual; p.relu = a.relu_in != 0;
  p.TH = TH; p.TW = TW; p.mtiles = mtiles; p.ntiles = a.cout / BN;
  p.grid = ((mtiles + 7) / 8) * 8 * p.ntiles * (dual ? 2 : nph);
  p.ntiles_out = mtiles * nph;
  p.stat_to_acc = a.stat_acc != nullptr;
  const int BNk = dual ? 128 : BN;
  const int epi = 256 * (BNk + 8) * 2 + 4 * BNk * 8;
  const int use6 = gi_opt(GI_OPT_IGEMM6), use8 = use6 ? gi_opt(GI_OPT_IGEMM8) : 0;
  const bool fits31 = in_px * a.ldin * 2 < (1ll << 31) && (int64_t)a.cout * (mode == 1 ? 4 : (mode == 2 ? 9 : 16)) * a.cin * 2 * (dual ? 2 : 1) < (1ll << 31);
  const bool take8 = use8 && (mode != 2 || (TW == 32 && !a.relu_in)) && (dual || BN == 128 || mode == 2) && a.cin % (mode == 0 ? 64 : 32) == 0 && TW >= 16 &&
      fits31 && !(mode == 0 && a.relu_in) && (use8 >= 2 || p.grid >= gi_tune("GI_IGEMM8_MINGRID", 512));
  p.bwd_range = a.bwd_c > 0 && (a.bwd_c0 != 0 || a.bwd_c != a.cout);
  if (a.bwd_acc && !a.mask && mode != 2 && a.cout % 128 == 0 && BN == 128 && (!p.bwd_range || (take8 && a.bwd_c0 % 128 == 0 && a.bwd_c % 128 == 0 && a.bwd_c0 + a.bwd_c <= a.cout))) {
    const int64_t px_per_tile = 256 * (mode == 1 ? 4 : 1);
    GI_REQUIRE(a.bwd_ldx % 8 == 0 && out_px * a.bwd_ldx < (1ll << 31) && (a.bwd_pg == 0 || a.bwd_pg % px_per_tile == 0) && a.coffout == 0,
               "igemm5: fused BatchNorm-backward reduction: layout");
    p.take_bwd = true;
  }
  if (take8) {
    if (mode == 2 && a.pool2 && !a.mask && !a.stat_acc && !a.partials) {
      GI_REQUIRE(a.coffout == 0 && (int64_t)a.n * (a.Hs / 2) * (a.Ws / 2) * a.ldout < (1ll << 31), "igemm8: pooled output layout");
      p.take_pool = true;
    }
    p.take_mask_bits = dual && !a.relu_in && a.mask && a.mask_bits && a.cout == 64 && !a.bias && a.act_out == GI_ACT_NONE && !a.stat_acc && !a.partials;
    p.take_c1w = p.take_mask_bits && a.c1w_part && a.c1w_img && mtiles % 8 == 0 && a.c1w_part_floats >= (int64_t)p.grid * 1024 &&
                 (int64_t)a.n * 16 * a.Hs * a.Ws < (1ll << 31);
    p.family = GI_FAM_IGEMM8;
    p.variant = mode == 2 ? (BN == 64 ? 7 : 6) : (dual ? 2 : mode) * 2 + (p.relu ? 1 : 0);
    p.lds_bytes = p.variant == 7 ? 2 * 22528 + 4 * 4096 : (mode == 2 ? 2 * 22528 : 2 * 20480) + 4 * 8192;
    p.lds_attr_bytes = p.lds_bytes;
    p.name = name8(p.variant);
  } else if (use6 && mode != 2 && fits31 && !(mode == 0 && a.relu_in)) {
    const int lds6 = 2 * 320 * 128 + 4 * BNk * 128;
    p.family = GI_FAM_IGEMM6;
    p.variant = (dual ? 4 : (BN == 64 ? 2 : 0) + mode) * 2 + (p.relu ? 1 : 0);
    p.lds_bytes = lds6 > epi ? lds6 : epi;
    p.lds_attr_bytes = 160 * 1024;
    p.name = name6(p.variant);
  } else {
    const int ring = 2 * (mode == 2 ? 384 : 320) * 128 + 3 * BNk * 128;
    p.family = GI_FAM_IGEMM5;
    p.variant = dual ? 6 : (BN == 64 ? 3 : 0) + mode;
    p.lds_bytes = ring > epi ? ring : epi;
    p.lds_attr_bytes = 160 * 1024;
    p.name = name5(p.variant);
  }
  return GI_OK;
}

int plan_igemm3(int mode, const IgemmArgs& a, IgemmPlan& p) {
  const int M = a.n * a.Hs * a.Ws;
  const int nph = mode == 1 ? 4 : 1;
  int BN = (a.cout % 128 == 0) ? 128 : 64;
  if (mode != 2) {
    const int tiles = ((M + 255) / 256) * (a.cout / BN) * nph;
    if (tiles < 128) return NEXT;
    if (gi_tune("GI_IGEMM3_NARROW", 1) && BN == 128 && tiles < 256) BN = 64;
  }
  GI_REQUIRE(!a.stat_acc || a.stat_pg == 0 || a.stat_pg % 256 == 0, "igemm3: stat_pg=%d must be a multiple of 256", a.stat_pg);
  const int64_t in_px = (int64_t)M * (mode == 0 ? 4 : 1), out_px = (int64_t)M * nph;
  GI_REQUIRE(in_px * a.ldin < (1ll << 31) && out_px * a.ldout < (1ll << 31), "igemm3: tensor too large for 32-bit offsets");
// ... 53 lines not shown
  if (p.pf != 2 && p.pf != 4) p.pf = 1;
  p.nw = (p.fold || gi_opt(GI_OPT_IGEMM7_WAVES) == 4) ? 4 : 8;
  const int ring = p.nstg * (128 + BN) * 128, epi = 128 * (BN + 8) * 2 + 4 * BN * 8;
  p.lds_bytes = ring > epi ? ring : epi;
  p.lds_attr_bytes = 144 * 1024;
  p.stat_to_acc = a.stat_acc != nullptr;
  p.ntiles_out = mtiles * nph;
  p.name = name7(p.variant + (p.fold ? 4 : 0));
  return GI_OK;
}

int plan_generic(int dtype, int mode, const IgemmArgs& a, IgemmPlan& p) {
  if (dtype != GI_F16 && dtype != GI_F32) { gi_set_error("igemm: bad dtype %d", dtype); return GI_ERR_INVALID; }
  const bool f16 = dtype == GI_F16;
  const int EPC = f16 ? 8 : 4, BK = 8 * EPC;
  GI_REQUIRE(a.cin % BK == 0, "igemm: cin=%d must be a multiple of %d", a.cin, BK);
  GI_REQUIRE(a.cout % 64 == 0, "igemm: cout=%d must be a multiple of 64", a.cout);
  GI_REQUIRE(a.ldin % EPC == 0 && a.coffin % EPC == 0 && a.ldout % EPC == 0 && a.coffout % EPC == 0,
             "igemm: leading dims / channel offsets must be 16-byte aligned");
  const int phases = mode ? 4 : 1, M = a.n * a.Hs * a.Ws;
  const int nk = (mode ? 4 : 16) * a.cin / BK;
  const int64_t in_elems = (int64_t)M * (mode ? 1 : 4) * a.ldin, out_pixels = (int64_t)M * phases;
  GI_REQUIRE(in_elems < (1ll << 31) && out_pixels * a.ldout < (1ll << 31), "igemm: tensor too large for 32-bit offsets");
  const bool wide = (a.cout % 128 == 0);
  int BM = wide ? 128 : 256, BN = wide ? 128 : 64;
  int mt = (M + BM - 1) / BM, nt = a.cout / BN;
  int tiles = mt * nt * phases;
  int splitk = 1;
  int fix_max = gi_tune("GI_IGEMM_FIX_MAXSPLIT", 8);
  if (fix_max < 2) fix_max = 8;
  bool fixup = gi_opt(GI_OPT_IGEMM_FIXUP) && a.tickets && a.ws && a.force_splitk == 0 && tiles < 256 && nk >= 8;
  bool half_n = false;
  if (fixup) {
    if (wide && tiles * fix_max < 256) { half_n = true; BN = 64; nt = a.cout / BN; tiles = mt * nt * phases; }
    splitk = (256 + tiles - 1) / tiles;
    if (splitk > fix_max) splitk = fix_max;
    if (splitk > nk / 4) splitk = nk / 4;
    if (splitk < 1) splitk = 1;
    if (tiles > GI_IGEMM_TICKETS || a.ws_bytes < (int64_t)splitk * tiles * BM * BN * 4) {
      fixup = false; splitk = 1;
      if (half_n) { half_n = false; BN = 128; nt = a.cout / BN; tiles = mt * nt * phases; }
    }
  }
  if (fixup) {
  } else if (a.force_splitk > 0) splitk = a.force_splitk;
  else if (tiles < 256 && nk >= 8) {
    splitk = (gi_tune("GI_IGEMM_SPLIT_BLOCKS", 384) + tiles - 1) / tiles;
    if (splitk > nk / 4) splitk = nk / 4;
    if (splitk > 64) splitk = 64;
    if (splitk < 1) splitk = 1;
  }
  if (splitk > 1 && (a.ws == nullptr || a.ws_bytes < out_pixels * a.cout * 4)) splitk = 1;
  p.kt_per_split = (nk + splitk - 1) / splitk;
  p.splitk = (nk + p.kt_per_split - 1) / p.kt_per_split;
  p.fixup = fixup && p.splitk > 1;
  p.finish_launch = p.splitk > 1 && !p.fixup;
  p.atomics_ws = p.finish_launch && a.ws_bytes < (int64_t)p.splitk * out_pixels * a.cout * 4;
  GI_REQUIRE(!a.stat_acc || a.stat_pg == 0 || a.stat_pg % 256 == 0, "igemm: stat_pg=%d must be a multiple of 256", a.stat_pg);
  p.family = GI_FAM_GENERIC; p.mode = mode ? 1 : 0; p.bn = BN; p.BM = BM; p.half_n = half_n;
  p.mtiles = mt; p.ntiles = nt; p.grid = mt * nt * phases * p.splitk;
  p.stat_to_acc = a.stat_acc != nullptr;
  p.ntiles_out = mt * phases;
  if (p.finish_launch) {
    const int RL = 256 / (a.cout / 4) > 0 ? 256 / (a.cout / 4) : 1;
    int rpb = 64;
    while (rpb > RL && (out_pixels + rpb - 1) / rpb < 256) rpb >>= 1;
    if (rpb < RL) rpb = RL;
    GI_REQUIRE(a.cout <= 1024, "igemm split-K finish: cout=%d > 1024", a.cout);
    p.finish_rows = rpb; p.finish_blocks = (int)((out_pixels + rpb - 1) / rpb);
    p.stat_to_acc = a.stat_acc && !a.partials;
    p.ntiles_out = p.finish_blocks;
  }
  p.name = f16 ? (p.fixup ? "igemm<f16,fixup>" : (p.splitk > 1 ? "igemm<f16,splitk>" : "igemm<f16>"))
               : (p.fixup ? "igemm<f32,fixup>" : (p.splitk > 1 ? "igemm<f32,splitk>" : "igemm<f32>"));
  return GI_OK;
}

}

int gi_igemm_plan(int dtype, int mode, const IgemmArgs& a, IgemmPlan* p) {
  *p = IgemmPlan{};
  const bool dma = mode == 2 || (dtype == GI_F16 && a.force_splitk == 0 && gi_opt(GI_OPT_IGEMM_VARIANT) >= 3);
  int rc = NEXT;
  if (dma && a.cin % 64 == 0 && a.cout % 64 == 0 && a.cin <= 2048) {
    const int use5 = gi_opt(GI_OPT_IGEMM5);
    if ((mode == 1 && (use5 & 1)) || (mode == 0 && (use5 & 2)) || (mode == 2 && (use5 & 4))) rc = plan_halo(mode, a, *p);
    if (rc == NEXT) rc = plan_igemm3(mode, a, *p);
  }
  if (rc == NEXT && mode == 2) return GI_ERR_UNSUPPORTED;
  if (rc == NEXT && dma) rc = plan_igemm7(mode, a, *p);
  if (rc == NEXT) rc = plan_generic(dtype, mode, a, *p);
  return rc;
}

int op_igemm(hipStream_t st, int dtype, int mode, IgemmArgs& a) {
  IgemmPlan p;
  GI_TRY(gi_igemm_plan(dtype, mode, a, &p));
  switch (p.family) {
    case GI_FAM_IGEMM3: GI_TRY(launch_igemm3(st, p, a)); break;
    case GI_FAM_IGEMM5: case GI_FAM_IGEMM6: GI_TRY(launch_igemm5(st, p, a)); break;
    case GI_FAM_IGEMM7: GI_TRY(launch_igemm7(st, p, a)); break;
    case GI_FAM_IGEMM8: GI_TRY(launch_igemm8(st, p, a)); break;
    default: GI_TRY(launch_igemm(st, dtype, p, a)); break;
  }
  gi_note_kernel(p.name);
  if (p.fold) gi_note_fold();
  gi_igemm_returns(p, a);
  return GI_OK;
}

void gi_igemm_returns(const IgemmPlan& p, IgemmArgs& a) {
  a.stat_used = p.stat_to_acc ? 1 : 0;
  a.ntiles_out = p.ntiles_out;
  if (p.family == GI_FAM_IGEMM7) a.fold_applied = p.fold ? 1 : 0;
  if (p.family == GI_FAM_IGEMM5 || p.family == GI_FAM_IGEMM6 || p.family == GI_FAM_IGEMM8) {
    if (p.take_mask) a.mask_applied = 1;
    if (p.take_bwd) a.bwd_applied = 1;
    a.c1w_applied = p.take_c1w ? 1 : 0; a.c1w_blocks = p.take_c1w ? p.grid : 0;
    a.pool_applied = p.take_pool ? 1 : 0;
  }
}
```

### gan-inpainting_amd/csrc/net.hip

```cpp
#include <string>
#include <vector>
#include <string.h>

#include "common.h"
#include "stat_acc.h"

namespace {

struct TensorDesc {
  std::string name;
  int kind;
  int64_t shape[4];
  int ndim;
  int64_t offset, numel;
};

struct Conv {
  int ca = 0, cb = 0;
  int64_t w_off = -1, bias_off = -1;
  int64_t packed_off = -1, phase_off = -1;
  int64_t inf_off = -1;
};
struct BN {
  int c = 0;
// ... 697 lines not shown
  net->drop_counter = 0;
  return GI_OK;
}
extern "C" int gi_net_get_dropout_state(gi_net* net, uint64_t* seed, uint64_t* counter) {
  GI_REQUIRE(net && seed && counter, "get_dropout_state: null");
  *seed = net->drop_seed;
  *counter = net->drop_counter;
  return GI_OK;
}
extern "C" int gi_net_set_dropout_state(gi_net* net, uint64_t seed, uint64_t counter) {
  GI_REQUIRE(net, "set_dropout_state: null");
  net->drop_seed = seed;
  net->drop_counter = counter;
  return GI_OK;
}
extern "C" int gi_net_dropout_mask(gi_net* net, int slot, int level, uint8_t* out_nchw, int64_t count) {
  GI_REQUIRE(net && net->kind == 0 && net->bound, "dropout_mask: generator handle required");
  GI_REQUIRE(slot >= 0 && slot < net->n_slots && level >= 5 && level <= net->nd - 1, "dropout_mask: slot=%d level=%d", slot, level);
  const int n = net->slot_n[slot], c = net->ch[level - 1], hw = net->Hk[level - 1] * net->Wk[level - 1];
  GI_REQUIRE(count == (int64_t)n * c * hw, "dropout_mask: count %lld != %lld", (long long)count, (long long)n * c * hw);
  return op_mask_nchw_to_nhwc(net->ctx->stream, (const uint8_t*)net->slot(slot, net->oMask[level]), out_nchw, n, c, hw, 0);
}
extern "C" int gi_net_set_dropout_mask(gi_net* net, int slot, int level, const uint8_t* mask_nchw) {
  GI_REQUIRE(net && net->kind == 0, "set_dropout_mask: generator handle required");
  GI_REQUIRE(slot >= 0 && slot < net->n_slots && level >= 5 && level <= net->nd - 1, "set_dropout_mask: slot=%d level=%d", slot, level);
  net->ext_mask[slot][level] = mask_nchw;
  return GI_OK;
}

namespace {

struct BNPtrs { float *scale, *shift, *mean, *inv; };
BNPtrs bn_ptrs(const gi_net* net, int slot, const BN& b, int group = 0) {
  float* base = (float*)net->slot(slot, net->oStats) + b.stat_off + (int64_t)group * 4 * b.c;
  return {base, base + b.c, base + 2 * b.c, base + 3 * b.c};
}

struct Slice { const void* p = nullptr; int c = 0, ld = 0, coff = 0; };
Slice sl(const void* p, int c, int ld = 0, int coff = 0) { return {p, c, ld ? ld : c, coff}; }
void* concat_buf(const gi_net* net, int s, int k) { return net->slot(s, net->oC[k]); }
Slice concat(const gi_net* net, int s, int k) { return sl(concat_buf(net, s, k), 2 * net->ch[k]); }
Slice skip_half(const gi_net* net, int s, int k) { return sl(concat_buf(net, s, k), net->ch[k], 2 * net->ch[k], 0); }
Slice up_half(const gi_net* net, int s, int k) { return sl(concat_buf(net, s, k), net->ch[k], 2 * net->ch[k], net->ch[k]); }
Slice up_input(const gi_net* net, int s, int k) { return k == net->nd ? sl(net->slot(s, net->oE), net->ch[k]) : concat(net, s, k); }

struct StatPlan { unsigned long long* acc = nullptr; unsigned long long* zero_next = nullptr; int zero_words = 0; int pg = 0; int reps = 1; bool use = false; };
int stat_reps_for(int64_t adders) {
  int r = 1;
  while (r < GI_STAT_MAXREP && adders > 256 * r) r <<= 1;
  return r;
}
StatPlan stat_plan(const gi_net* net, const BN& b, int64_t gemm_rows, int64_t tile_rows, int train) {
  StatPlan sp;
  const int g = net->kind == 1 ? net->bn_groups : 1;
  if (!train || !net->use_acc || b.acc_off < 0 || (g == 2 && (gemm_rows % 2 != 0 || (gemm_rows / 2) % 256 != 0))) return sp;
  unsigned long long* base = (unsigned long long*)net->shared(net->oAcc) + b.acc_off;
  sp.use = true;
  sp.reps = stat_reps_for(tile_rows);
  sp.acc = base + b.fwd_par * b.acc_block();
  sp.zero_next = base + (b.fwd_par ^ 1) * b.acc_block();
  sp.zero_words = (int)gi_stat_block_words(b.c, b.dirty[b.fwd_par ^ 1]);
  sp.pg = g == 2 ? (int)(gemm_rows / 2) : 0;
  return sp;
}

BnAccArgs bn_acc_args(const gi_net* net, int slot, const BN& b, const StatPlan& sp, int64_t pg, int g) {
  BNPtrs p = bn_ptrs(net, slot, b, 0);
  BnAccArgs a;
  a.acc = sp.acc; a.gamma = net->params + b.gamma_off; a.beta = net->params + b.beta_off;
  a.running_mean = net->buffers + b.rmean_off; a.running_var = net->buffers + b.rvar_off;
  a.scale = p.scale; a.shift = p.shift; a.save_mean = p.mean; a.save_invstd = p.inv;
  a.count = pg; a.momentum = 0.1f; a.eps = 1e-5f; a.groups = g; a.out_stride = 4 * b.c;
  a.zero_next = sp.zero_words > 0 ? sp.zero_next : nullptr; a.zero_words = sp.zero_words;
  a.reps = sp.reps;
  return a;
}
void bn_acc_commit(gi_net* net, int slot, const BN& b, const StatPlan& sp) {
  b.dirty[b.fwd_par ^ 1] = 0;
  b.dirty[b.fwd_par] = sp.reps;
  b.fwd_par ^= 1;
  if (b.id >= 0) net->eval_gen[slot][b.id] = 0;
}

struct Dropout { uint8_t* mask = nullptr; float scale = 1.f; uint64_t seed = 0; float p = 0.f; };
int dropout_draw(gi_net* net, Dropout& d, int64_t count) {
  GI_TRY(op_fill_dropout(net->ctx->stream, d.mask, count, d.seed, d.p));
  d.p = 0.f;
  return GI_OK;
}
int dropout_prepare(gi_net* net, int s, int k, int n, bool defer, Dropout& d) {
  d = Dropout();
  if (!net->train || !(net->dropout_p > 0.f) || k < 5 || k > net->nd - 1) return GI_OK;
  const int co = net->ch[k - 1], hw = net->Hk[k - 1] * net->Wk[k - 1];
  d.mask = (uint8_t*)net->slot(s, net->oMask[k]);
  d.scale = 1.f / (1.f - net->dropout_p);
  if (net->ext_mask[s][k]) return op_mask_nchw_to_nhwc(net->ctx->stream, net->ext_mask[s][k], d.mask, n, co, hw, 1);
  d.seed = net->drop_seed + 0x1000003ull * (++net->drop_counter);
  d.p = net->dropout_p;
  return defer ? GI_OK : dropout_draw(net, d, (int64_t)n * hw * co);
}

struct SideCopy { const void* src = nullptr; void* dst = nullptr; int64_t bytes = 0; };
SideCopy input_side_copy(const gi_net* net, int s, const float* x, int n, const StatPlan& sp) {
  const int64_t bytes = (int64_t)n * net->H * net->W * 4;
  if (!sp.use || bytes % 16 != 0) return SideCopy();
  return {x, net->slot(s, net->oX), bytes};
}
int input_copy(gi_net* net, int s, const float* x, int n) {
  GI_HIP(hipMemcpyAsync(net->slot(s, net->oX), x, (size_t)n * net->H * net->W * 4, hipMemcpyDeviceToDevice, net->ctx->stream));
  return GI_OK;
}

struct BnOpts { bool apply = true; Dropout drop; SideCopy side; };
int bn_forward(gi_net* net, int slot, const BN& b, const void* raw, int64_t pixels, int ntiles, Slice dst, int act, int train,
               const StatPlan& sp, const BnOpts& o = BnOpts()) {
  hipStream_t st = net->ctx->stream;
  const int g = net->kind == 1 ? net->bn_groups : 1;
  const int64_t pg = pixels / g;
  const size_t T = net->tsz();
  const Dropout& drop = o.drop;
  if (sp.use) {
    const BnAccArgs a = bn_acc_args(net, slot, b, sp, pg, g);
    bn_acc_commit(net, slot, b, sp);
    if (o.apply) return op_bn_apply_acc(st, net->dtype, raw, (void*)dst.p, pixels, b.c, dst.ld, dst.coff, act, drop.mask, drop.scale, drop.seed, drop.p, a,
                                        o.side.src, o.side.dst, o.side.bytes);
    return op_bn_finalize_acc(st, b.c, a);
  }
  const bool aligned = g == 1 || (pg % 256 == 0 && ntiles % g == 0);
  if (g == 2 && aligned) {
    BNPtrs p = bn_ptrs(net, slot, b, 0);
    const int rows = ntiles / 2;
    GI_TRY(op_bn_finalize(st, (const float*)net->shared(net->oPart), rows, b.c, pg, net->params + b.gamma_off, net->params + b.beta_off,
                          net->buffers + b.rmean_off, net->buffers + b.rvar_off, p.scale, p.shift, p.mean, p.inv, train, 0.1f, 1e-5f, 2,
                          (int64_t)rows * 2 * b.c, 4 * b.c));
    if (o.apply) GI_TRY(op_bn_apply(st, net->dtype, raw, (void*)dst.p, pixels, b.c, dst.ld, dst.coff, p.scale, p.shift, act, drop.mask, drop.scale, pg, 4 * b.c));
    return GI_OK;
  }
  for (int j = 0; j < g; ++j) {
    BNPtrs p = bn_ptrs(net, slot, b, j);
    const char* rj = (const char*)raw + (int64_t)j * pg * b.c * T;
    const float* part = (const float*)net->shared(net->oPart);
    int rows = ntiles / g;
    if (aligned) {
      part += (int64_t)j * rows * 2 * b.c;
    } else {
      float* scratch = (float*)net->shared(net->oPart) + (int64_t)ntiles * 2 * b.c;
      GI_REQUIRE((int64_t)ntiles * 2 * b.c + (pg / 32 + 8) * 2 * b.c <= net->part_floats, "internal: partials buffer too small for a column pass");
      GI_TRY(op_col_stats(st, net->dtype, rj, pg, b.c, scratch, &rows));
      part = scratch;
    }
    const bool cached = !train && g == 1 && b.id >= 0 && net->eval_gen[slot][b.id] == net->affine_gen;
    if (!cached) {
      GI_TRY(op_bn_finalize(st, part, rows, b.c, pg, net->params + b.gamma_off, net->params + b.beta_off, net->buffers + b.rmean_off,
                            net->buffers + b.rvar_off, p.scale, p.shift, p.mean, p.inv, train, 0.1f, 1e-5f));
      if (b.id >= 0) net->eval_gen[slot][b.id] = (!train && g == 1) ? net->affine_gen : 0;
    }
    if (o.apply)
      GI_TRY(op_bn_apply(st, net->dtype, rj, (char*)dst.p + (int64_t)j * pg * dst.ld * T, pg, b.c, dst.ld, dst.coff, p.scale, p.shift, act,
                         drop.mask ? drop.mask + (int64_t)j * pg * b.c : nullptr, drop.scale));
  }
  return GI_OK;
}

BwdFuse bwd_fuse_plan(gi_net* net, int slot, const BN& bn, const void* x, int64_t pixels, int64_t gemm_tiles, float slope) {
  BwdFuse f;
  const int on = gi_opt(GI_OPT_BN_BWD_FUSE);
// ... 375 lines not shown
  void* D = side_dz(net);
  const void* D1 = lrelu1_done ? a1.g1 : D;
  if (!lrelu1_done) GI_TRY(act_bn_bwd(net, s, a1, D));
  if (need_wgrad) GI_TRY(bias_grad(net, cv, D1, a1.pixels, c));
  if (need_wgrad && c1w && c1w->applied)
    GI_TRY(op_c1_wgrad_reduce(st, c1w->part, dW, c * 16, c1w->blocks, c1w->part + (int64_t)c1w->blocks * 1024,
                              net->c1w_floats - (int64_t)c1w->blocks * 1024));
  else if (need_wgrad)
    GI_TRY(op_c1_wgrad(st, dt, D1, (const float*)net->slot(s, net->oX), dW, n, Hs, Ws, c, c, 0, 0, iLS, 1.f, nullptr,
                       (float*)net->shared(net->oPart), net->part_floats));
  if (dx) GI_TRY(op_c1_scatter(st, dt, D1, net->params + cv.w_off, nullptr, dx, n, Hs, Ws, c, c, 0, 0, 0, iLS, net->shared(net->oCol)));
  return GI_OK;
}

int unet_forward_inference(gi_net* net, int s, const float* x, float* y, int n) {
  hipStream_t st = net->ctx->stream;
  const int nd = net->nd, dt = net->dtype;
  if (net->inf_gen != net->affine_gen) GI_TRY(unet_sync_inference(net));
  net->slot_n[s] = n;
  net->slot_train[s] = 0;
  net->slot_inference[s] = 1;
  net->slot_fused_u2[s] = 0;
  auto shift = [&](const BN& b) { return (const float*)net->shared(b.inf_off) + b.c; };
  GI_TRY(op_c1_gather(st, dt, x, net->params + net->conv[1].w_off, concat_buf(net, s, 1), n, net->Hk[1], net->Wk[1], net->ch[1], 2 * net->ch[1], 0,
                      GI_ACT_LRELU, 1.f));
  for (int k = 2; k < nd; ++k) {
    Gemm g = gemm_args(net, skip_half(net, s, k - 1), net->shared(net->conv[k].inf_off), skip_half(net, s, k), n, net->Hk[k], net->Wk[k]);
    g.a.act_out = GI_ACT_LRELU; g.a.bias = shift(net->dnorm[k]);
    GI_TRY(gemm_run(net, 0, g));
  }
  {
    Gemm g = gemm_args(net, skip_half(net, s, nd - 1), packed_ptr(net, net->conv[nd]), up_input(net, s, nd), n, net->Hk[nd], net->Wk[nd]);
    g.a.act_out = GI_ACT_RELU;
    GI_TRY(gemm_run(net, 0, g));
  }
  for (int k = nd; k >= 2; --k) {
    Gemm g = gemm_args(net, up_input(net, s, k), net->shared(net->up[k].inf_off), up_half(net, s, k - 1), n, net->Hk[k], net->Wk[k]);
    if (k < nd) { g.a.relu_in = 1; g.a.relu_cend = net->ch[k]; }
    g.a.act_out = GI_ACT_RELU; g.a.bias = shift(net->unorm[k]);
    GI_TRY(gemm_run(net, 1, g));
  }
  return head_forward(net, s, y, n, false);
}

int plain_norm_forward(gi_net* net, int slot, const BN& b, const void* raw, int n, int hw, Slice dst, int act, const Dropout& drop = Dropout()) {
  hipStream_t st = net->ctx->stream;
  if (net->norm_kind == 1)
    return op_in_forward(st, net->dtype, raw, (void*)dst.p, n, hw, b.c, dst.ld, dst.coff, act, drop.mask, drop.scale, 1e-5f,
                         (float*)net->slot(slot, net->oInStats) + b.in_off);
  return op_bn_apply(st, net->dtype, raw, (void*)dst.p, (int64_t)n * hw, b.c, dst.ld, dst.coff, nullptr, nullptr, act, drop.mask, drop.scale);
}

int unet_forward_plain(gi_net* net, int s, const float* x, float* y, int n);
int unet_backward_plain(gi_net* net, int s, const float* dy, float* dx, int need_wgrad, int phase);

IgemmFold fold_offer(const gi_net* net, int s, const BN& b, const StatPlan& sp, int64_t pixels, Slice dst, int act, const Dropout& drop = Dropout()) {
  IgemmFold fold;
  fold.bn = bn_acc_args(net, s, b, sp, pixels, 1);
  fold.dst = (void*)dst.p; fold.lddst = dst.ld; fold.coffdst = dst.coff; fold.act = act;
  fold.drop_mask = drop.mask; fold.drop_scale = drop.scale; fold.drop_seed = drop.seed; fold.drop_p = drop.p;
  return fold;
}

int unet_forward(gi_net* net, int s, const float* x, float* y, int n) {
  hipStream_t st = net->ctx->stream;
  const int nd = net->nd, dt = net->dtype, train = net->train;
  if (net->norm_kind != 0) return unet_forward_plain(net, s, x, y, n);
  if (!train && net->inference && nd >= 3) return unet_forward_inference(net, s, x, y, n);
  net->slot_inference[s] = 0;
  if (train) ++net->affine_gen;
  net->slot_n[s] = n;
  net->slot_train[s] = train;
  const bool fuse_u2 = nd >= 3 && net->out_c == 1 && net->fuse_head && op_c1_affine_ok(dt, 2 * net->ch[1], net->Wk[1], 2 * net->ch[1], 0);
  net->slot_fused_u2[s] = fuse_u2 ? 1 : 0;
  GI_TRY(op_c1_gather(st, dt, x, net->params + net->conv[1].w_off, concat_buf(net, s, 1), n, net->Hk[1], net->Wk[1], net->ch[1], 2 * net->ch[1], 0,
                      GI_ACT_LRELU, 1.f, nullptr, gi_opt(GI_OPT_MASK_BITS) ? (unsigned long long*)net->slot(s, net->oBits1) : nullptr, &net->slot_bits1[s]));
  bool x_saved = false;
  for (int k = 2; k < nd; ++k) {
    const int64_t pix = (int64_t)n * net->Hk[k] * net->Wk[k];
    void* R = net->slot(s, net->oR[k]);
    StatPlan sp = stat_plan(net, net->dnorm[k], pix, (pix + 127) / 128, train);
    const bool offer = sp.use && dt == GI_F16;
    IgemmFold fold;
    if (offer) fold = fold_offer(net, s, net->dnorm[k], sp, pix, skip_half(net, s, k), GI_ACT_LRELU);
    Gemm g = gemm_args(net, skip_half(net, s, k - 1), packed_ptr(net, net->conv[k]), sl(R, net->ch[k]), n, net->Hk[k], net->Wk[k]);
    with_stats(net, g, sp, offer ? &fold : nullptr);
    GI_TRY(gemm_run(net, 0, g));
    if (g.a.fold_applied) { bn_acc_commit(net, s, net->dnorm[k], sp); continue; }
    BnOpts o;
    if (k == 2) o.side = input_side_copy(net, s, x, n, sp);
    GI_TRY(bn_forward(net, s, net->dnorm[k], R, pix, g.a.ntiles_out, skip_half(net, s, k), GI_ACT_LRELU, train, sp, o));
    if (o.side.bytes > 0) x_saved = true;
  }
  {
    Gemm g = gemm_args(net, skip_half(net, s, nd - 1), packed_ptr(net, net->conv[nd]), up_input(net, s, nd), n, net->Hk[nd], net->Wk[nd]);
    g.a.act_out = GI_ACT_RELU;
    GI_TRY(gemm_run(net, 0, g));
  }
  BnAccArgs u2_acc;
  bool u2_deferred = false;
  if (!x_saved) GI_TRY(input_copy(net, s, x, n));
  for (int k = nd; k >= 2; --k) {
    const int64_t pix = (int64_t)n * net->Hk[k] * net->Wk[k], opix = 4 * pix;
    void* U = net->slot(s, net->oU[k]);
    StatPlan sp = stat_plan(net, net->unorm[k], pix, (pix + 127) / 128 * 4, train);
    Dropout drop;
    GI_TRY(dropout_prepare(net, s, k, n, true, drop));
    const bool fused = (k == 2) && fuse_u2;
    const bool offer = sp.use && dt == GI_F16 && !fused;
    IgemmFold fold;
    if (offer) fold = fold_offer(net, s, net->unorm[k], sp, opix, up_half(net, s, k - 1), GI_ACT_RELU, drop);
    Gemm g = gemm_args(net, up_input(net, s, k), phase_ptr(net, net->up[k]), sl(U, net->ch[k - 1]), n, net->Hk[k], net->Wk[k]);
    if (k < nd) { g.a.relu_in = 1; g.a.relu_cend = net->ch[k]; }
    with_stats(net, g, sp, offer ? &fold : nullptr);
    GI_TRY(gemm_run(net, 1, g));
    if (g.a.fold_applied) { bn_acc_commit(net, s, net->unorm[k], sp); continue; }
    if (drop.p > 0.f && !sp.use) GI_TRY(dropout_draw(net, drop, opix * net->ch[k - 1]));
    if (fused && sp.use) {
      u2_acc = bn_acc_args(net, s, net->unorm[k], sp, opix, 1);
      bn_acc_commit(net, s, net->unorm[k], sp);
      u2_deferred = true;
      continue;
    }
    BnOpts o;
    o.apply = !fused; o.drop = drop;
    GI_TRY(bn_forward(net, s, net->unorm[k], U, opix, g.a.ntiles_out, up_half(net, s, k - 1), GI_ACT_RELU, train, sp, o));
  }
  C1Affine aff = u2_affine(net, s);
  if (u2_deferred) aff.bn = &u2_acc;
  return head_forward(net, s, y, n, true, fuse_u2 ? &aff : nullptr);
}

int unet_backward(gi_net* net, int s, const float* dy, float* dx, int need_wgrad, int phase) {
  if (net->norm_kind != 0) return unet_backward_plain(net, s, dy, dx, need_wgrad, phase);
  const int nd = net->nd, n = net->slot_n[s];
  GI_REQUIRE(n > 0 && (net->slot_train[s] || !need_wgrad), "unet_backward: slot %d holds no train-mode forward", s);
  GI_REQUIRE(!net->slot_inference[s], "unet_backward: slot %d holds an inference forward (gi_net_set_inference): nothing was saved for a backward", s);
  GI_REQUIRE(net->out_c == 1 || !need_wgrad, "unet_backward: parameter gradients of a %d-channel generator are not built", net->out_c);
  const int evalbn = net->slot_train[s] ? 0 : 1;
  net->bwd_eval = evalbn;
  auto gC = [&](int k) { return (void*)net->shared(net->ogC[k]); };
  auto gA = [&](int k) { return (void*)net->shared(net->ogA[k]); };
  auto dropped = [&](int k) { return !evalbn && net->dropout_p > 0.f && k >= 5 && k <= nd - 1; };
  void* D = nullptr;
  if (phase == 0 || phase == 1) {
    C1Affine aff = u2_affine(net, s);
    GI_TRY(head_backward(net, s, dy, need_wgrad, net->slot_fused_u2[s] ? &aff : nullptr));
    GI_TRY(clear_pending_bwd(net, &net->unorm[2], nd - 1));
    for (int k = 1; k <= nd - 1; ++k) {
      const int kk = k + 1, ck = net->ch[k], ca = net->up[kk].ca;
      const int64_t pix = (int64_t)n * net->Hk[k] * net->Wk[k];
      D = side_dz(net);
      BwdFuse& pend = net->bwd_pending[net->unorm[kk].id];
      ActBnBwdArgs b = act_bwd_args(up_half(net, s, k), pix, GI_ACT_NONE);
      set_g2(b, sl(gC(k), ck, 2 * ck, ck));
      b.x = net->slot(s, net->oU[kk]);
      if (dropped(kk)) b.drop_scale = 1.f / (1.f - net->dropout_p);
      GI_TRY(act_bn_bwd(net, s, b, D, &net->unorm[kk], need_wgrad, &pend));
      pend = BwdFuse();
      if (need_wgrad) {
        WgradArgs wa = wgrad_args(net, up_input(net, s, kk), sl(D, ck), n, net->Hk[kk], net->Wk[kk], net->grads + net->up[kk].w_off);
        wa.relu_S = kk < nd ? 1 : 0;
        GI_TRY(wgrad_run(net, wa));
      }
      void* gout = (kk == nd) ? (void*)net->shared(net->ogE) : gC(kk);
      Gemm g = gemm_args(net, sl(D, ck), packed_ptr(net, net->up[kk]), sl(gout, ca), n, net->Hk[kk], net->Wk[kk]);
      const int kn = kk + 1;
      if (kk <= nd - 1 && !dropped(kn)) {
        const int64_t pixn = (int64_t)n * net->Hk[kk] * net->Wk[kk];
        BwdFuse& bf = net->bwd_pending[net->unorm[kn].id];
        bf = bwd_fuse_plan(net, s, net->unorm[kn], net->slot(s, net->oU[kn]), pixn, pixn / 256, 0.f);
        bf.c0 = ca / 2; bf.c = ca / 2;
        with_bn_bwd(g, bf);
      }
      GI_TRY(gemm_run(net, 0, g));
    }
  }
  if (phase == 1) return GI_OK;
  const bool run_inner = phase != 4, run_outer = phase != 3;
  int lrelu1_done = 0;
  C1WFuse c1w;
  if (run_inner) {
    const int c = net->ch[nd], cb = net->ch[nd - 1];
    D = side_dz(net);
    ActBnBwdArgs b = act_bwd_args(up_input(net, s, nd), (int64_t)n * net->Hk[nd] * net->Wk[nd], GI_ACT_NONE);
    set_g2(b, sl(net->shared(net->ogE), c));
    GI_TRY(act_bn_bwd(net, s, b, D));
    if (need_wgrad)
      GI_TRY(wgrad_run(net, wgrad_args(net, sl(D, c), skip_half(net, s, nd - 1), n, net->Hk[nd], net->Wk[nd], net->grads + net->conv[nd].w_off)));
    GI_TRY(gemm_run(net, 1, gemm_args(net, sl(D, c), phase_ptr(net, net->conv[nd]), sl(gA(nd - 1), cb), n, net->Hk[nd], net->Wk[nd])));
  }
  for (int k = nd - 1; k >= 2; --k) {
    if (k >= 5 ? !run_inner : !run_outer) continue;
    const int c = net->ch[k], cb = net->ch[k - 1];
    D = side_dz(net);
    ActBnBwdArgs b = act_bwd_args(skip_half(net, s, k), (int64_t)n * net->Hk[k] * net->Wk[k], GI_ACT_LRELU);
    set_g1(b, sl(gA(k), c));
    set_g2(b, sl(gC(k), c, 2 * c));
// ... 550 lines not shown
```

### include/ganinpaint.h

```cpp
#ifndef GANINPAINT_H
#define GANINPAINT_H

#include <stddef.h>
#include <stdint.h>

#ifdef __cplusplus
extern "C" {
#endif

typedef enum {
  GI_OK = 0,
  GI_ERR_INVALID = -1,
  GI_ERR_HIP = -2,
  GI_ERR_STATE = -3,
  GI_ERR_UNSUPPORTED = -4
} gi_status;

typedef enum { GI_F32 = 0, GI_F16 = 1 } gi_dtype;
typedef enum { GI_ACT_NONE = 0, GI_ACT_RELU = 1, GI_ACT_LRELU = 2 } gi_act;

typedef struct gi_ctx gi_ctx;
typedef struct gi_net gi_net;

const char* gi_last_error(void);
int gi_version(void);

int gi_set_option(const char* name, int value);
int gi_get_option(const char* name, int* value);
const char* gi_debug_last_kernel(void);
int gi_debug_fold_count(void);

int gi_ctx_create(int device_id, void* hip_stream, gi_ctx** out);
int gi_ctx_destroy(gi_ctx* ctx);
int gi_ctx_sync(gi_ctx* ctx);

int gi_unet_create(gi_ctx* ctx, int num_downs, int ngf, float dropout_p, int H, int W, int max_n,
                   int dtype, int n_slots, gi_net** out);
int gi_unet_create_ex(gi_ctx* ctx, int num_downs, int ngf, int out_c, float dropout_p, int H, int W,
                      int max_n, int dtype, int n_slots, gi_net** out);
int gi_unet_create_norm(gi_ctx* ctx, int num_downs, int ngf, int out_c, int norm_kind, float dropout_p, int H,
                        int W, int max_n, int dtype, int n_slots, gi_net** out);
int gi_unet_create_padded(gi_ctx* ctx, int num_downs, int ngf, int ch1, int out_c, int norm_kind, float dropout_p,
                          int H, int W, int max_n, int dtype, int n_slots, gi_net** out);
int gi_patchgan_create(gi_ctx* ctx, int H, int W, int sigmoid, int max_n, int dtype, int n_slots,
                       gi_net** out);
int gi_patchgan_create_sn(gi_ctx* ctx, int H, int W, int sigmoid, int spectral_norm, int n_power_iterations, int max_n,
                          int dtype, int n_slots, gi_net** out);
int gi_net_sn_read(gi_net* net, int slot, float* sigma6, float* eff_params, int64_t count);
int gi_dcgan_create(gi_ctx* ctx, int H, int W, int max_n, int dtype, int n_slots, gi_net** out);
int gi_dcgan_debug_forward_convs(gi_net* net, int slot, const float* x, int n);
int gi_net_destroy(gi_net* net);

int gi_net_tensor_count(gi_net* net);
int gi_net_tensor_desc(gi_net* net, int index, char* name, int name_cap, int* kind, int64_t* shape4,
                       int* ndim, int64_t* offset, int64_t* numel);
int64_t gi_net_param_floats(gi_net* net);
int64_t gi_net_buffer_floats(gi_net* net);
int64_t gi_net_workspace_bytes(gi_net* net);
int gi_net_bind(gi_net* net, float* params, float* grads, float* buffers, void* workspace,
                int64_t workspace_bytes);
int gi_net_sync_weights(gi_net* net);
int gi_net_set_train(gi_net* net, int train);
int gi_net_set_inference(gi_net* net, int inference);
int gi_net_set_loss_scale(gi_net* net, float scale);
int gi_net_set_bn_groups(gi_net* net, int groups);
int gi_net_set_dropout_seed(gi_net* net, uint64_t seed);
int gi_net_get_dropout_state(gi_net* net, uint64_t* seed, uint64_t* counter);
int gi_net_set_dropout_state(gi_net* net, uint64_t seed, uint64_t counter);
int gi_net_dropout_mask(gi_net* net, int slot, int level, uint8_t* out_nchw, int64_t count);
int gi_net_set_dropout_mask(gi_net* net, int slot, int level, const uint8_t* mask_nchw);

int gi_net_saved_activation(gi_net* net, int slot, int kind, int level, float* out_nchw, int64_t count);
int gi_net_debug_nonzero_tickets(gi_net* net, int* count);

int gi_net_forward(gi_net* net, int slot, const float* x, float* y, int n);
int gi_net_backward(gi_net* net, int slot, const float* dy, float* dx, int need_wgrad);

int gi_net_backward_phase(gi_net* net, int slot, const float* dy, float* dx, int need_wgrad, int phase);
int64_t gi_net_phase_split(gi_net* net);
int64_t gi_net_phase_split2(gi_net* net);

typedef struct gi_comm gi_comm;
int gi_comm_unique_id(char* id128_host);
int gi_comm_create(const char* id128_host, int rank, int world, int device_id, gi_comm** out);
int gi_comm_destroy(gi_comm* comm);
int gi_allreduce_sum_f32(gi_comm* comm, float* buf, int64_t count, void* hip_comm_stream);
int gi_net_allreduce_grads_async(gi_net* net, gi_comm* comm, int64_t begin, int64_t end, void* hip_comm_stream);
int gi_allreduce_wait(gi_comm* comm, void* hip_comm_stream, void* hip_compute_stream);

int gi_patchgan_gradient_penalty(gi_net* net, const float* xhat, int n, float lam, float* penalty_out);
int gi_patchgan_gp_saved_activation(gi_net* net, int level, float* out_nchw, int64_t count);
int gi_interpolate(gi_ctx* ctx, const float* real, const float* fake, const float* eps, int n, int64_t hw, float* out);

int gi_mask_apply(gi_ctx* ctx, const float* ground, const float* mask, float* mask_c, float* masked,
                  int64_t count, int flags);
int gi_mask_composite(gi_ctx* ctx, const float* masked, const float* gen, const float* mask_c,
                      float* inpainted, int64_t count);
int gi_mul(gi_ctx* ctx, const float* a, const float* b, float* out, int64_t count);
int gi_add(gi_ctx* ctx, const float* a, const float* b, float* out, int64_t count, float alpha);

int gi_loss_l1(gi_ctx* ctx, const float* a, const float* b, int64_t count, float* loss_out,
               float* grad_a, float gscale, float* scratch);
int gi_loss_rmse(gi_ctx* ctx, const float* a, const float* b, int64_t count, float eps, float* loss_out,
                 float* grad_a, float gscale, float* scratch);
int gi_loss_mse(gi_ctx* ctx, const float* a, const float* b, int64_t count, float* loss_out,
                float* grad_a, float gscale, float* scratch);
int gi_loss_local(gi_ctx* ctx, const float* yhat, const float* y, const float* mask, int64_t count,
                  int kind, float* loss_out, float* grad_yhat, float gscale, float* scratch);
int gi_loss_adv(gi_ctx* ctx, const float* pred, int n, int kind, float target, float* loss_out,
                float* grad_pred, float gscale);
int gi_loss_adv_pair(gi_ctx* ctx, const float* pred2, int n_each, int kind, float target_a, float target_b, float* loss_a,
                     float* loss_b, float* grad_pred2, float gscale_a, float gscale_b);

// ... 124 lines not shown
                    const int64_t* flip_keys_dev, uint64_t flip_seed, int out_kind, void* out);

int gi_diffaug_params(gi_ctx* ctx, int policy, uint64_t seed, uint64_t key0, int n, int H, int W, void* table);
int gi_diffaug_fwd(gi_ctx* ctx, const float* x, const void* table, int n, int H, int W, int colour, float* y);
int gi_diffaug_bwd(gi_ctx* ctx, const float* dy, const void* table, int n, int H, int W, int colour, float* dx);
int gi_diffaug_apply(gi_ctx* ctx, int policy, uint64_t seed, uint64_t key0, const float* x, int n, int H, int W, float* y);
int gi_diffaug_apply_bwd(gi_ctx* ctx, int policy, uint64_t seed, uint64_t key0, const float* dy, int n, int H, int W, float* dx);

int gi_conv_s2_forward(gi_ctx* ctx, int dtype, const void* in, const void* w_packed, void* out,
                       int n, int H, int W, int cb, int ldin, int ca, int ldout, int relu_in,
                       int act_out, float* ws, int64_t ws_bytes);
int gi_convT_s2_forward(gi_ctx* ctx, int dtype, const void* in, const void* w_phase, void* out,
                        int n, int H, int W, int ca, int ldin, int cb, int ldout, int relu_in,
                        int act_out, float* ws, int64_t ws_bytes);
typedef struct gi_igemm_ex {
  int relu_cend;
  const void* mask; int ldmask; float mask_slope;
  const void* add; int ldadd;
  const unsigned long long* mask_bits;
  unsigned long long* stat_acc; int stat_reps; int stat_pg;
  float* partials;
  const void* bwd_x; int bwd_ldx;
  const float* bwd_scale; const float* bwd_shift; const float* bwd_mean; const float* bwd_inv; int bwd_stride;
  float bwd_slope; unsigned long long* bwd_acc; int bwd_reps; int64_t bwd_pg;
  int bwd_c0, bwd_c;
  int mask_applied, bwd_applied, stat_used, ntiles_out;
} gi_igemm_ex;
int gi_conv_s2_forward_ex(gi_ctx* ctx, int dtype, const void* in, const void* w_packed, void* out,
                          int n, int H, int W, int cb, int ldin, int ca, int ldout, int relu_in,
                          int act_out, float* ws, int64_t ws_bytes, gi_igemm_ex* ex);
int gi_convT_s2_forward_ex(gi_ctx* ctx, int dtype, const void* in, const void* w_phase, void* out,
                           int n, int H, int W, int ca, int ldin, int cb, int ldout, int relu_in,
                           int act_out, float* ws, int64_t ws_bytes, gi_igemm_ex* ex);
typedef struct gi_igemm_plan_info {
  char name[48];
  int grid, splitk, ntiles_out;
  int mask_applied, bwd_applied, stat_used, c1w_applied, c1w_blocks, pool_applied, fold_applied;
} gi_igemm_plan_info;
int gi_debug_igemm_plan(int dtype, int mode, int n, int Hs, int Ws, int cin, int ldin, int cout, int ldout, int relu_in,
                        int act_out, int64_t ws_bytes, int has_tickets, const gi_igemm_ex* ex, int offered,
                        gi_igemm_plan_info* out);
int64_t gi_stat_acc_words(int c);
int gi_stat_acc_read(gi_ctx* ctx, const unsigned long long* acc, int c, int reps, int group, double* out_dev);
int gi_wgrad_s2(gi_ctx* ctx, int dtype, const void* S, const void* L, float* dW, int n, int Hs, int Ws,
                int ca, int ldS, int cb, int ldL, int relu_S, float scale);
int64_t gi_wgrad_s2_scratch_bytes(int dtype, int n, int Hs, int Ws, int ca, int cb);
int gi_wgrad_s2_ws(gi_ctx* ctx, int dtype, const void* S, const void* L, float* dW, int n, int Hs, int Ws,
                   int ca, int ldS, int cb, int ldL, int relu_S, float scale, float* scratch, int64_t scratch_bytes);
int gi_c1_gather(gi_ctx* ctx, int dtype, const float* img, const float* w, void* out, int n, int Hs, int Ws, int c,
                 int ldout, int coffout, int act_out, float in_scale, const float* bias, unsigned long long* bits,
                 int* bits_written);
int gi_c1_scatter(gi_ctx* ctx, int dtype, const void* X, const float* w, const float* bias, float* img, int n, int Hs,
                  int Ws, int c, int ldx, int coffx, int relu_in, int post, float out_scale, void* col_scratch,
                  float* img2, const void* x2, int ld2, const float* scale2, const float* shift2);
int gi_c1_wgrad(gi_ctx* ctx, int dtype, const void* X, const float* img, float* dW, int n, int Hs, int Ws, int c, int ldx,
                int coffx, int relu_in, float scale, float img_scale, const void* x2, int ld2, const float* scale2,
                const float* shift2, float* scratch, int64_t scratch_floats);
int gi_c1_wgrad_reduce(gi_ctx* ctx, const float* part, float* dW, int count, int blocks, float* scratch,
                       int64_t scratch_floats);
int64_t gi_c1_head4_col_bytes(int n, int Hs, int Ws);
int gi_c1_head4_forward(gi_ctx* ctx, const void* X, const float* w, const float* bias, float* out, float* out2, int n,
                        int Hs, int Ws, int ldx, int coffx, int relu_in, void* col_scratch);
int gi_c1_head4_dgrad(gi_ctx* ctx, const float* g, const float* w, void* out, int n, int Hs, int Ws, int ldout,
                      int coffout);
int gi_debug_col_stats(gi_ctx* ctx, int dtype, const void* x, int64_t pixels, int c, float* partials, int* rows_out);
int gi_debug_bn_finalize(gi_ctx* ctx, const float* partials, int rows, int c, int64_t count, const float* gamma,
                         const float* beta, float* running_mean, float* running_var, float* scale, float* shift,
                         float* save_mean, float* save_invstd, int train, float momentum, float eps, int groups,
                         int64_t part_stride, int out_stride);
int gi_debug_bn_apply(gi_ctx* ctx, int dtype, const void* x, void* y, int64_t pixels, int c, int ldy, int coffy,
                      const float* scale, const float* shift, int act, const uint8_t* drop_mask, float drop_scale, int64_t pg,
                      int gstride);
typedef struct gi_bn_acc_args {
  const unsigned long long* acc; int reps;
  const float* gamma; const float* beta;
  float* running_mean; float* running_var;
  float* scale; float* shift; float* save_mean; float* save_invstd;
  int64_t count;
  float momentum, eps;
  int groups, out_stride;
  unsigned long long* zero_next; int zero_words;
} gi_bn_acc_args;
int gi_debug_bn_finalize_acc(gi_ctx* ctx, int c, const gi_bn_acc_args* b);
int gi_debug_bn_apply_acc(gi_ctx* ctx, int dtype, const void* x, void* y, int64_t pixels, int c, int ldy, int coffy, int act,
                          uint8_t* drop_mask, float drop_scale, uint64_t drop_seed, float drop_p, const gi_bn_acc_args* b,
                          const void* side_src, void* side_dst, int64_t side_bytes);
typedef struct gi_act_bn_bwd_args {
  const void* g1; int ldg1, coffg1;
  const void* g2; int ldg2, coffg2;
  const void* y; int ldy, coffy;
  const void* x;
  void* dx;
  int64_t pixels; int c;
  int act; float drop_scale;
  int has_bn, eval_bn;
  const float* gamma; const float* save_mean; const float* save_invstd;
  float* dgamma; float* dbeta; float inv_loss_scale;
  float* partials;
  float* sums;
  const float* fwd_scale; const float* fwd_shift;
  int groups, stat_stride;
  unsigned long long* acc; int acc_reps;
  unsigned long long* zero_next; int zero_words;
  int reduce_done;
} gi_act_bn_bwd_args;
int gi_debug_act_bn_bwd(gi_ctx* ctx, int dtype, const gi_act_bn_bwd_args* a);
int gi_debug_in_forward(gi_ctx* ctx, int dtype, const void* x, void* y, int n, int hw, int c, int ldy, int coffy, int act,
                        const uint8_t* drop_mask, float drop_scale, float eps, float* stats);
int gi_debug_act_in_bwd(gi_ctx* ctx, int dtype, const gi_act_bn_bwd_args* a, int n, int hw, const float* stats);
int gi_debug_bias_grad(gi_ctx* ctx, int dtype, const void* dz, int64_t pixels, int c, float scale, float* dbias, float* partials);
int gi_debug_tanh_bwd(gi_ctx* ctx, const float* dy, const float* y, float* dx, int64_t count, float scale);
int gi_debug_fill_dropout(gi_ctx* ctx, uint8_t* mask_nhwc, int64_t count, uint64_t seed, float p);
int gi_debug_mask_layout(gi_ctx* ctx, const uint8_t* src, uint8_t* dst, int n, int c, int hw, int to_nhwc);
int gi_debug_mul_slope(gi_ctx* ctx, int dtype, const void* tin, const void* a, void* tout, int64_t count);
int gi_debug_bn_tangent_inject(gi_ctx* ctx, int dtype, const void* dta, const void* y, const void* tx, const void* x, void* dxp,
                               int64_t pixels, int c, const float* gamma, const float* mean, const float* inv, float* dgamma,
                               float dgamma_scale, float* partials, float* sums);
int gi_debug_gp_direction(gi_ctx* ctx, const float* g, int n, int64_t hw, float lam, float* sumsq, float* amax, float* v,
                          float* penalty, float* sc);
int gi_debug_gp_unscale_add(gi_ctx* ctx, const float* src, const float* sc, float* dst, int64_t count);
int gi_debug_sn_power_iteration(gi_ctx* ctx, const float* w, int ca, int K, int cb, float* u, float* v, int iters, int train,
                                float* sigma_out);
int gi_debug_sn_project_add(gi_ctx* ctx, const float* g, const float* w_eff, const float* u, const float* v, const float* sigma,
                            int ca, int K, int cb, const float* scale_dev, float* dst);
int gi_debug_stat_acc_add(gi_ctx* ctx, unsigned long long* acc, int c, int reps, int group, int q, const float* addends,
                          int rows);
typedef struct gi_pack_job {
  const float* w; void* packed; void* phase;
  int ca, cb, scale_on_b;
  const float* scale;
} gi_pack_job;
int gi_debug_pack_weights_batch(gi_ctx* ctx, int dtype, const gi_pack_job* jobs, int n);
typedef struct gi_head_args {
  const void* a4; const float* w5; const float* wl; const float* bl;
  float* h; float* out;
  int n, Hh, Wh, c, sigmoid;
  float* out2;
  const float* scale4; const float* shift4; int n_per_group, gstride;
  float* tbuf; int64_t tbuf_bytes;
  const gi_bn_acc_args* bn;
} gi_head_args;
typedef struct gi_head_bwd_args {
  const void* a4; const float* w5; const float* wl; const float* h; const float* out;
  const float* dy;
  void* da4;
  float* dw5; float* dwl; float* dbl;
  float* dh;
  int n, Hh, Wh, c, sigmoid;
  float loss_scale;
  float* scratch; int64_t scratch_bytes;
  const float* scale4; const float* shift4; int n_per_group, gstride;
  const void* bwd_x;
  const float* bwd_scale; const float* bwd_shift; const float* bwd_mean; const float* bwd_inv;
  int bwd_stride, bwd_n_per_group, bwd_reps; float bwd_slope;
  unsigned long long* bwd_acc;
  int bwd_applied;
} gi_head_bwd_args;
int gi_debug_head_forward(gi_ctx* ctx, int dtype, const gi_head_args* a);
int gi_debug_head_backward(gi_ctx* ctx, int dtype, gi_head_bwd_args* a);
int64_t gi_debug_head_scratch_bytes(int max_n, int Hh, int Wh);
int gi_debug_vgg_conv3x3(gi_ctx* ctx, const void* in, const float* w, void* w_packed, void* out, int n, int H, int W, int cin,
                         int cout, int transposed, const float* bias, int act_out, int pool2, const void* mask, const void* add,
                         int* pool_applied, int* mask_applied);
int gi_debug_vgg_conv1(gi_ctx* ctx, const float* xa, const float* xb, int n, int H, int W, const float* w, const float* bias,
                       float* w1, void* out);
int gi_debug_vgg_maxpool2(gi_ctx* ctx, const void* in, void* out, int nimg, int Ho, int Wo, int C);
// ... 37 lines not shown
```

Before: 17340 images/sec.

## Add channel-owner small-map conv kernel with fused batchnorm epilogue for deep U-Net layers

Adds a dedicated kernel for the deep U-Net layers where the spatial map holds at most 128 pixels. Each workgroup owns a 16-channel output slice and runs the whole K reduction. The BN batch statistics, affine, activation and dropout are computed in the kernel epilogue, replacing separate stat accumulation and apply passes. It also skips dead filter taps on tiny maps. The aim is to cut launch count and the poor occupancy of the generic implicit GEMM on these tiny layers. The cost is low parallelism (cout/16 workgroups) and a long serial K loop per block.

After: 17230 images/sec. No clear change (-0.6%).

```diff
diff --git a/gan-inpainting_amd/backend.py b/gan-inpainting_amd/backend.py
--- a/gan-inpainting_amd/backend.py
+++ b/gan-inpainting_amd/backend.py
@@ -19,6 +19,7 @@
     "gi_get_option": (_i, [C.c_char_p, C.POINTER(_i)]),
     "gi_debug_last_kernel": (C.c_char_p, []),
     "gi_debug_fold_count": (_i, []),
+    "gi_debug_smallmap_count": (_i, [_i]),
     "gi_ctx_create": (_i, [_i, _vp, C.POINTER(_vp)]),
     "gi_ctx_destroy": (_i, [_vp]),
     "gi_ctx_sync": (_i, [_vp]),
@@ -194,6 +195,7 @@
     "gi_debug_bn_finalize": (_i, [_vp, _vp, _i, _i, _i64, _vp, _vp, _vp, _vp, _vp, _vp, _vp, _vp, _i, _f, _f, _i, _i64, _i]),
     "gi_debug_bn_apply": (_i, [_vp, _i, _vp, _vp, _i64, _i, _i, _i, _vp, _vp, _i, _vp, _f, _i64, _i]),
     "gi_debug_bn_finalize_acc": (_i, [_vp, _i, _vp]),
+    "gi_debug_smallmap_forward": (_i, [_vp, _i, _vp, _vp, _vp, _i, _i, _i, _i, _i, _i, _i, _i, _i, _i, _i, _vp, _vp, _i, _i, _i, _vp, _f, _u64, _f]),
     "gi_debug_bn_apply_acc": (_i, [_vp, _i, _vp, _vp, _i64, _i, _i, _i, _i, _vp, _f, _u64, _f, _vp, _vp, _vp, _i64]),
     "gi_debug_act_bn_bwd": (_i, [_vp, _i, _vp]),
     "gi_debug_in_forward": (_i, [_vp, _i, _vp, _vp, _i, _i, _i, _i, _i, _i, _vp, _f, _f, _vp]),
diff --git a/gan-inpainting_amd/csrc/api.hip b/gan-inpainting_amd/csrc/api.hip
--- a/gan-inpainting_amd/csrc/api.hip
+++ b/gan-inpainting_amd/csrc/api.hip
@@ -23,12 +23,14 @@
   {"GI_IGEMM5", 7, 0, 0}, {"GI_IGEMM6", 1, 0, 0}, {"GI_IGEMM7", 1, 0, 0}, {"GI_IGEMM_FIXUP", 1, 0, 0}, {"GI_IGEMM_VARIANT", 3, 0, 0},
   {"GI_BN_ACC", 1, 0, 0}, {"GI_FUSE_HEAD", 1, 0, 0}, {"GI_HEAD_FAST", 1, 0, 0}, {"GI_BN_BWD_FUSE", 1, 0, 0}, {"GI_BN_BWD_SMALL", 512, 0, 0},
   {"GI_WGRAD2", 1, 0, 0}, {"GI_WGRAD3", 1, 0, 0}, {"GI_IGEMM8", 1, 0, 0}, {"GI_BN_FOLD", 0, 0, 0}, {"GI_C1_FUSED", 1, 0, 0},
-  {"GI_WGRAD_STREAM", 1, 0, 0}, {"GI_MASK_BITS", 1, 0, 0}, {"GI_C1W_FUSE", 1, 0, 0}, {"GI_IGEMM7_WAVES", 8, 0, 0},
+  {"GI_WGRAD_STREAM", 1, 0, 0}, {"GI_MASK_BITS", 1, 0, 0}, {"GI_C1W_FUSE", 1, 0, 0}, {"GI_IGEMM7_WAVES", 8, 0, 0}, {"GI_SMALLMAP", 1, 0, 0},
 };
 thread_local const char* g_last_kernel = "";
 int g_fold_count = 0;
+int g_smallmap_count[2] = {0, 0};
 }
 void gi_note_fold() { __atomic_fetch_add(&g_fold_count, 1, __ATOMIC_RELAXED); }
+void gi_note_smallmap(bool bn) { __atomic_fetch_add(&g_smallmap_count[bn ? 1 : 0], 1, __ATOMIC_RELAXED); }
 
 int gi_opt(int id) {
   OptDesc& o = g_opts[id];
@@ -63,6 +65,7 @@
 }
 const char* gi_debug_last_kernel(void) { return g_last_kernel; }
 int gi_debug_fold_count(void) { return __atomic_load_n(&g_fold_count, __ATOMIC_RELAXED); }
+int gi_debug_smallmap_count(int with_bn) { return __atomic_load_n(&g_smallmap_count[with_bn ? 1 : 0], __ATOMIC_RELAXED); }
 
 const char* gi_last_error(void) { return g_err; }
 int gi_version(void) { return 100; }
@@ -205,6 +208,11 @@
   if ((offered & 2) && a.mask_bits) { a.c1w_img = (const float*)dummy; a.c1w_part = (float*)dummy; a.c1w_part_floats = (int64_t)1 << 40; a.c1w_scale = 1.f; }
   if (offered & 4) a.pool2 = 1;
   if (offered & 8) a.bias = (const float*)dummy;
+  IgemmFold sm_bn = {};
+  if (offered & 16) {
+    a.smallmap_offer = 1;
+    if (a.stat_acc) { sm_bn.bn.groups = 1; sm_bn.lddst = ldout; sm_bn.act = GI_ACT_RELU; a.smallmap_bn = &sm_bn; }
+  }
   IgemmPlan p;
   GI_TRY(gi_igemm_plan(dtype, mode, a, &p));
   gi_igemm_returns(p, a);
@@ -394,6 +402,41 @@
   return op_bn_apply(ctx->stream, dtype, x, y, pixels, c, ldy, coffy, scale, shift, act, drop_mask, drop_scale, pg, gstride);
 }
 
+int gi_debug_smallmap_forward(gi_ctx* ctx, int mode, const void* in, const void* w, void* out, int n, int Hs, int Ws, int cin, int ldin, int cout,
+                              int ldout, int coffout, int relu_in, int relu_cend, int act_out, const gi_bn_acc_args* bn, void* dst, int lddst,
+                              int coffdst, int act, uint8_t* drop_mask, float drop_scale, uint64_t drop_seed, float drop_p) {
+  GI_REQUIRE(ctx && in && w && out && (mode == 0 || mode == 1) && n >= 1 && Hs >= 1 && Ws >= 1, "debug_smallmap_forward: bad argument");
+  GI_REQUIRE(dbg_act_ok(act_out) && relu_cend >= 0 && relu_cend % 64 == 0 && relu_cend <= cin, "debug_smallmap_forward: act_out=%d relu_cend=%d", act_out, relu_cend);
+  IgemmArgs a;
+  memset(&a, 0, sizeof(a));
+  a.in = in; a.w = w; a.out = out;
+  a.n = n; a.Hs = Hs; a.Ws = Ws;
+  a.cin = cin; a.ldin = ldin; a.cout = cout; a.ldout = ldout; a.coffout = coffout;
+  a.relu_in = relu_in; a.relu_cend = relu_cend; a.act_out = act_out;
+  a.smallmap_offer = 1;
+  IgemmFold f = {};
+  if (bn) {
+    GI_REQUIRE(bn->gamma && bn->beta && bn->running_mean && bn->running_var && bn->scale && bn->shift && bn->save_mean && bn->save_invstd && dst,
+               "debug_smallmap_forward: null pointer");
+    GI_REQUIRE(dbg_act_ok(act) && bn->groups == 1 && bn->count == (int64_t)n * Hs * Ws * (mode == 1 ? 4 : 1), "debug_smallmap_forward: act=%d groups=%d count=%lld",
+               act, bn->groups, (long long)bn->count);
+    GI_REQUIRE(drop_p >= 0.f && drop_p < 1.f && (drop_p == 0.f || drop_mask), "debug_smallmap_forward: drop_p=%g needs a mask to store the draw", (double)drop_p);
+    f.bn.gamma = bn->gamma; f.bn.beta = bn->beta; f.bn.running_mean = bn->running_mean; f.bn.running_var = bn->running_var;
+    f.bn.scale = bn->scale; f.bn.shift = bn->shift; f.bn.save_mean = bn->save_mean; f.bn.save_invstd = bn->save_invstd;
+    f.bn.count = bn->count; f.bn.momentum = bn->momentum; f.bn.eps = bn->eps; f.bn.groups = 1; f.bn.out_stride = bn->out_stride; f.bn.reps = 1;
+    f.dst = dst; f.lddst = lddst; f.coffdst = coffdst; f.act = act;
+    f.drop_mask = drop_mask; f.drop_scale = drop_scale; f.drop_seed = drop_seed; f.drop_p = drop_p;
+    a.smallmap_bn = &f;
+  }
+  IgemmPlan p;
+  GI_TRY(gi_igemm_plan(GI_F16, mode, a, &p));
+  if (p.family != GI_FAM_SMALLMAP) {
+    gi_set_error("debug_smallmap_forward: the channel-owner kernel does not serve this layer (%s would)", p.name);
+    return GI_ERR_UNSUPPORTED;
+  }
+  return op_igemm(ctx->stream, GI_F16, mode, a);
+}
+
 int gi_debug_bn_finalize_acc(gi_ctx* ctx, int c, const gi_bn_acc_args* b) {
   GI_REQUIRE(ctx && c >= 1, "debug_bn_finalize_acc: bad argument");
   BnAccArgs o;
diff --git a/gan-inpainting_amd/csrc/bn_acc.h b/gan-inpainting_amd/csrc/bn_acc.h
--- a/gan-inpainting_amd/csrc/bn_acc.h
+++ b/gan-inpainting_amd/csrc/bn_acc.h
@@ -23,13 +23,8 @@
 __device__ __forceinline__ void zero_words64(unsigned long long* p, int n) {
   for (int i = threadIdx.x; i < n; i += 256) p[i] = 0ull;
 }
-template <bool COHERENT = false>
-__device__ __forceinline__ void bn_from_acc(const BnAccP& a, int c, int ch, int j, bool write, float& sc_out, float& sh_out) {
-  const float gam = a.gamma[ch], bet = a.beta[ch];
-  float rm = 0.f, rv = 0.f;
-  if (write) { rm = a.rmean[ch]; rv = a.rvar[ch]; }
-  double t0, t1;
-  gi_stat_read2<COHERENT>(a.acc, c, a.reps, j, ch, t0, t1);
+__device__ __forceinline__ void bn_from_totals(const BnAccP& a, int ch, int j, bool write, double t0, double t1, float gam, float bet, float rm, float rv,
+                                               float& sc_out, float& sh_out) {
   const double m = t0 / a.count;
   double v = t1 / a.count - m * m;
   if (v < 0.0 || a.count <= 1.0) v = 0.0;
@@ -49,6 +44,15 @@
     a.sinv[o] = inv;
   }
 }
+template <bool COHERENT = false>
+__device__ __forceinline__ void bn_from_acc(const BnAccP& a, int c, int ch, int j, bool write, float& sc_out, float& sh_out) {
+  const float gam = a.gamma[ch], bet = a.beta[ch];
+  float rm = 0.f, rv = 0.f;
+  if (write) { rm = a.rmean[ch]; rv = a.rvar[ch]; }
+  double t0, t1;
+  gi_stat_read2<COHERENT>(a.acc, c, a.reps, j, ch, t0, t1);
+  bn_from_totals(a, ch, j, write, t0, t1, gam, bet, rm, rv, sc_out, sh_out);
+}
 
 __host__ __device__ __forceinline__ uint64_t gi_mix64(uint64_t z) {
   z = (z ^ (z >> 30)) * 0xBF58476D1CE4E5B9ull;
diff --git a/gan-inpainting_amd/csrc/common.h b/gan-inpainting_amd/csrc/common.h
--- a/gan-inpainting_amd/csrc/common.h
+++ b/gan-inpainting_amd/csrc/common.h
@@ -21,11 +21,12 @@
 
 enum gi_opt_id {
   GI_OPT_IGEMM5 = 0, GI_OPT_IGEMM6, GI_OPT_IGEMM7, GI_OPT_IGEMM_FIXUP, GI_OPT_IGEMM_VARIANT, GI_OPT_BN_ACC, GI_OPT_FUSE_HEAD,
-  GI_OPT_HEAD_FAST, GI_OPT_BN_BWD_FUSE, GI_OPT_BN_BWD_SMALL, GI_OPT_WGRAD2, GI_OPT_WGRAD3, GI_OPT_IGEMM8, GI_OPT_BN_FOLD, GI_OPT_C1_FUSED, GI_OPT_WGRAD_STREAM, GI_OPT_MASK_BITS, GI_OPT_C1W_FUSE, GI_OPT_IGEMM7_WAVES, GI_OPT_COUNT
+  GI_OPT_HEAD_FAST, GI_OPT_BN_BWD_FUSE, GI_OPT_BN_BWD_SMALL, GI_OPT_WGRAD2, GI_OPT_WGRAD3, GI_OPT_IGEMM8, GI_OPT_BN_FOLD, GI_OPT_C1_FUSED, GI_OPT_WGRAD_STREAM, GI_OPT_MASK_BITS, GI_OPT_C1W_FUSE, GI_OPT_IGEMM7_WAVES, GI_OPT_SMALLMAP, GI_OPT_COUNT
 };
 int gi_opt(int id);
 void gi_note_kernel(const char* name);
 void gi_note_fold();
+void gi_note_smallmap(bool bn);
 #ifdef GI_ABLATION
 #include <stdlib.h>
 static inline int gi_tune(const char* env, int dflt) { const char* e = getenv(env); return e ? atoi(e) : dflt; }
@@ -39,6 +40,14 @@
     static_for<N - 1>(f);
     f(std::integral_constant<int, N - 1>{});
   }
+}
+
+__device__ __forceinline__ h8_t relu7(h8_t v, short floor) {
+  typedef short s8_t __attribute__((ext_vector_type(8)));
+  s8_t h = __builtin_bit_cast(s8_t, v);
+  const s8_t z = {floor, floor, floor, floor, floor, floor, floor, floor};
+  h = __builtin_elementwise_max(h, z);
+  return __builtin_bit_cast(h8_t, h);
 }
 
 template <int ACT>
@@ -219,6 +228,7 @@
   int pool2, pool_applied;
   int stat_used;
   const IgemmFold* fold; int fold_applied;
+  int smallmap_offer; const IgemmFold* smallmap_bn; int smallmap_applied;
 };
 constexpr int GI_IGEMM_TICKETS = 1024;
 int op_igemm(hipStream_t st, int dtype, int mode, IgemmArgs& a);
diff --git a/gan-inpainting_amd/csrc/igemm7.hip b/gan-inpainting_amd/csrc/igemm7.hip
--- a/gan-inpainting_amd/csrc/igemm7.hip
+++ b/gan-inpainting_amd/csrc/igemm7.hip
@@ -32,13 +32,6 @@
   uint8_t* fdrop; float fdrop_scale; uint64_t fdrop_seed; uint32_t fdrop_thresh;
 };
 
-__device__ __forceinline__ h8_t relu7(h8_t v, short floor) {
-  typedef short s8_t __attribute__((ext_vector_type(8)));
-  s8_t h = __builtin_bit_cast(s8_t, v);
-  const s8_t z = {floor, floor, floor, floor, floor, floor, floor, floor};
-  h = __builtin_elementwise_max(h, z);
-  return __builtin_bit_cast(h8_t, h);
-}
 __device__ __forceinline__ void glds16_7(const char* src, char* lds_wave_base) {
   __builtin_amdgcn_global_load_lds((const __attribute__((address_space(1))) void*)src, (__attribute__((address_space(3))) void*)lds_wave_base,
                                    16, 0, 0);
diff --git a/gan-inpainting_amd/csrc/igemm_plan.h b/gan-inpainting_amd/csrc/igemm_plan.h
--- a/gan-inpainting_amd/csrc/igemm_plan.h
+++ b/gan-inpainting_amd/csrc/igemm_plan.h
@@ -1,7 +1,7 @@
 #pragma once
 #include "common.h"
 
-enum { GI_FAM_GENERIC = 0, GI_FAM_IGEMM3, GI_FAM_IGEMM5, GI_FAM_IGEMM6, GI_FAM_IGEMM7, GI_FAM_IGEMM8 };
+enum { GI_FAM_GENERIC = 0, GI_FAM_IGEMM3, GI_FAM_IGEMM5, GI_FAM_IGEMM6, GI_FAM_IGEMM7, GI_FAM_IGEMM8, GI_FAM_SMALLMAP };
 
 struct IgemmPlan {
   int family;
@@ -12,6 +12,7 @@
   int BM; bool half_n;
   int splitk, kt_per_split;
   bool fixup, finish_launch, atomics_ws;
+  bool smallmap_bn;
   bool fold, take_mask, take_mask_bits, take_c1w, take_bwd, bwd_range, take_pool, stat_to_acc;
   int TH, TW, mtiles, ntiles, grid, lds_bytes, lds_attr_bytes, ntiles_out;
   int finish_rows, finish_blocks;
@@ -26,6 +27,7 @@
 int launch_igemm5(hipStream_t st, const IgemmPlan& p, const IgemmArgs& a);
 int launch_igemm7(hipStream_t st, const IgemmPlan& p, const IgemmArgs& a);
 int launch_igemm8(hipStream_t st, const IgemmPlan& p, const IgemmArgs& a);
+int launch_smallmap(hipStream_t st, const IgemmPlan& p, const IgemmArgs& a);
 const char* gi_igemm3_zero_page(int dev);
 static inline const char* gi_igemm_zero_page() { int dev = 0; return hipGetDevice(&dev) == hipSuccess ? gi_igemm3_zero_page(dev) : nullptr; }
 
@@ -46,3 +48,8 @@
 #define GI_IGEMM8_KERNELS(X)  \
   X(7, 2, false, 64, "igemm8<2,64>") X(0, 0, false, 128, "igemm8<0>") X(1, 0, true, 128, "igemm8<0,relu>") X(2, 1, false, 128, "igemm8<1>") \
   X(3, 1, true, 128, "igemm8<1,relu>") X(4, 3, false, 128, "igemm8<3>") X(5, 3, true, 128, "igemm8<3,relu>") X(6, 2, false, 128, "igemm8<2>")
+#define GI_SMALLMAP_KERNELS(X)  \
+  X(0, 0, "smallmap<0>") X(1, 1, "smallmap<1>")
+#define GI_SMALLMAP_BN_NAMES(X) X(2, 0, "smallmap<0>+bn") X(3, 1, "smallmap<1>+bn")
+constexpr int GI_SMALLMAP_SLICE = 16;
+constexpr int GI_SMALLMAP_MAXPIX = 128;
diff --git a/gan-inpainting_amd/csrc/igemm_plan.hip b/gan-inpainting_amd/csrc/igemm_plan.hip
--- a/gan-inpainting_amd/csrc/igemm_plan.hip
+++ b/gan-inpainting_amd/csrc/igemm_plan.hip
@@ -12,6 +12,36 @@
 GI_NAME_FN(name6, GI_IGEMM6_KERNELS(GI_NAME4))
 GI_NAME_FN(name7, GI_IGEMM7_KERNELS(GI_NAME3) GI_IGEMM7_FOLD_NAMES(GI_NAME3))
 GI_NAME_FN(name8, GI_IGEMM8_KERNELS(GI_NAME4))
+#define GI_NAME2(V, A, NAME) case V: return NAME;
+GI_NAME_FN(name_sm, GI_SMALLMAP_KERNELS(GI_NAME2) GI_SMALLMAP_BN_NAMES(GI_NAME2))
+
+int plan_smallmap(int mode, const IgemmArgs& a, IgemmPlan& p) {
+  if (!a.smallmap_offer || mode == 2) return NEXT;
+  if (!gi_opt(GI_OPT_SMALLMAP) || gi_opt(GI_OPT_BN_FOLD) || !gi_opt(GI_OPT_IGEMM7) || gi_opt(GI_OPT_IGEMM7_WAVES) == 4) return NEXT;
+  if (a.cin % 64 != 0 || a.cout % 64 != 0) return NEXT;
+  const int64_t M = (int64_t)a.n * a.Hs * a.Ws, out_pixels = M * (mode == 1 ? 4 : 1), in_pixels = M * (mode == 0 ? 4 : 1);
+  if (M > GI_SMALLMAP_MAXPIX) return NEXT;
+  if (a.bias || a.mask || a.bwd_acc || a.pool2 || a.c1w_part || a.stat_pg != 0) return NEXT;
+  if (a.ldin % 8 != 0 || a.coffin % 8 != 0 || a.ldout % 4 != 0 || a.coffout % 4 != 0) return NEXT;
+  if (a.relu_in && a.relu_cend % 64 != 0) return NEXT;
+  const IgemmFold* f = a.smallmap_bn;
+  if (f) {
+    if (f->bn.groups != 1 || a.act_out != GI_ACT_NONE || f->lddst % 4 != 0 || f->coffdst % 4 != 0) return NEXT;
+    if (f->act != GI_ACT_RELU && f->act != GI_ACT_LRELU && f->act != GI_ACT_NONE) return NEXT;
+  } else if (a.stat_acc || a.partials) return NEXT;
+  p.family = GI_FAM_SMALLMAP; p.mode = mode; p.bn = GI_SMALLMAP_SLICE;
+  p.smallmap_bn = f != nullptr;
+  p.variant = mode + (f ? 2 : 0);
+  p.splitk = 1; p.kt_per_split = (mode == 1 ? 4 : 16) * a.cin / 64;
+  p.mtiles = 1; p.ntiles = a.cout / GI_SMALLMAP_SLICE; p.grid = p.ntiles;
+  p.nw = 4;
+  const int ring = 2 * ((((int)in_pixels + 7) & ~7) + 1) * 128, epi = 4 * 8 * 1024 + 1024;
+  p.lds_bytes = ring > epi ? ring : epi;
+  p.lds_attr_bytes = 2 * (4 * GI_SMALLMAP_MAXPIX + 1) * 128;
+  p.stat_to_acc = false; p.ntiles_out = 0;
+  p.name = name_sm(p.variant);
+  return GI_OK;
+}
 
 int plan_halo(int mode, const IgemmArgs& a, IgemmPlan& p) {
   if (!gi_is_pow2(a.Ws) || a.Ws < 8) return NEXT;
@@ -231,7 +261,8 @@
   *p = IgemmPlan{};
   const bool dma = mode == 2 || (dtype == GI_F16 && a.force_splitk == 0 && gi_opt(GI_OPT_IGEMM_VARIANT) >= 3);
   int rc = NEXT;
-  if (dma && a.cin % 64 == 0 && a.cout % 64 == 0 && a.cin <= 2048) {
+  if (dma && dtype == GI_F16) rc = plan_smallmap(mode, a, *p);
+  if (rc == NEXT && dma && a.cin % 64 == 0 && a.cout % 64 == 0 && a.cin <= 2048) {
     const int use5 = gi_opt(GI_OPT_IGEMM5);
     if ((mode == 1 && (use5 & 1)) || (mode == 0 && (use5 & 2)) || (mode == 2 && (use5 & 4))) rc = plan_halo(mode, a, *p);
     if (rc == NEXT) rc = plan_igemm3(mode, a, *p);
@@ -250,10 +281,12 @@
     case GI_FAM_IGEMM5: case GI_FAM_IGEMM6: GI_TRY(launch_igemm5(st, p, a)); break;
     case GI_FAM_IGEMM7: GI_TRY(launch_igemm7(st, p, a)); break;
     case GI_FAM_IGEMM8: GI_TRY(launch_igemm8(st, p, a)); break;
+    case GI_FAM_SMALLMAP: GI_TRY(launch_smallmap(st, p, a)); break;
     default: GI_TRY(launch_igemm(st, dtype, p, a)); break;
   }
   gi_note_kernel(p.name);
   if (p.fold) gi_note_fold();
+  if (p.family == GI_FAM_SMALLMAP) gi_note_smallmap(p.smallmap_bn);
   gi_igemm_returns(p, a);
   return GI_OK;
 }
@@ -262,6 +295,7 @@
   a.stat_used = p.stat_to_acc ? 1 : 0;
   a.ntiles_out = p.ntiles_out;
   if (p.family == GI_FAM_IGEMM7) a.fold_applied = p.fold ? 1 : 0;
+  a.smallmap_applied = p.family == GI_FAM_SMALLMAP ? 1 : 0;
   if (p.family == GI_FAM_IGEMM5 || p.family == GI_FAM_IGEMM6 || p.family == GI_FAM_IGEMM8) {
     if (p.take_mask) a.mask_applied = 1;
     if (p.take_bwd) a.bwd_applied = 1;
diff --git a/gan-inpainting_amd/csrc/net.hip b/gan-inpainting_amd/csrc/net.hip
--- a/gan-inpainting_amd/csrc/net.hip
+++ b/gan-inpainting_amd/csrc/net.hip
@@ -803,6 +803,10 @@
   if (b.id >= 0) net->eval_gen[slot][b.id] = 0;
 }
 
+void bn_smallmap_commit(gi_net* net, int slot, const BN& b) {
+  if (b.id >= 0) net->eval_gen[slot][b.id] = 0;
+}
+
 struct Dropout { uint8_t* mask = nullptr; float scale = 1.f; uint64_t seed = 0; float p = 0.f; };
 int dropout_draw(gi_net* net, Dropout& d, int64_t count) {
   GI_TRY(op_fill_dropout(net->ctx->stream, d.mask, count, d.seed, d.p));
@@ -1344,10 +1348,13 @@
     StatPlan sp = stat_plan(net, net->dnorm[k], pix, (pix + 127) / 128, train);
     const bool offer = sp.use && dt == GI_F16;
     IgemmFold fold;
-    if (offer) fold = fold_offer(net, s, net->dnorm[k], sp, pix, skip_half(net, s, k), GI_ACT_LRELU);
+    const bool small = train && dt == GI_F16;
+    if (offer || small) fold = fold_offer(net, s, net->dnorm[k], sp, pix, skip_half(net, s, k), GI_ACT_LRELU);
     Gemm g = gemm_args(net, skip_half(net, s, k - 1), packed_ptr(net, net->conv[k]), sl(R, net->ch[k]), n, net->Hk[k], net->Wk[k]);
     with_stats(net, g, sp, offer ? &fold : nullptr);
+    if (small) { g.a.smallmap_offer = 1; g.a.smallmap_bn = &fold; }
     GI_TRY(gemm_run(net, 0, g));
+    if (g.a.smallmap_applied) { bn_smallmap_commit(net, s, net->dnorm[k]); continue; }
     if (g.a.fold_applied) { bn_acc_commit(net, s, net->dnorm[k], sp); continue; }
     BnOpts o;
     if (k == 2) o.side = input_side_copy(net, s, x, n, sp);
@@ -1357,6 +1364,7 @@
   {
     Gemm g = gemm_args(net, skip_half(net, s, nd - 1), packed_ptr(net, net->conv[nd]), up_input(net, s, nd), n, net->Hk[nd], net->Wk[nd]);
     g.a.act_out = GI_ACT_RELU;
+    if (train && dt == GI_F16) g.a.smallmap_offer = 1;
     GI_TRY(gemm_run(net, 0, g));
   }
   BnAccArgs u2_acc;
@@ -1371,11 +1379,14 @@
     const bool fused = (k == 2) && fuse_u2;
     const bool offer = sp.use && dt == GI_F16 && !fused;
     IgemmFold fold;
-    if (offer) fold = fold_offer(net, s, net->unorm[k], sp, opix, up_half(net, s, k - 1), GI_ACT_RELU, drop);
+    const bool small = train && dt == GI_F16 && !fused;
+    if (offer || small) fold = fold_offer(net, s, net->unorm[k], sp, opix, up_half(net, s, k - 1), GI_ACT_RELU, drop);
     Gemm g = gemm_args(net, up_input(net, s, k), phase_ptr(net, net->up[k]), sl(U, net->ch[k - 1]), n, net->Hk[k], net->Wk[k]);
     if (k < nd) { g.a.relu_in = 1; g.a.relu_cend = net->ch[k]; }
     with_stats(net, g, sp, offer ? &fold : nullptr);
+    if (small) { g.a.smallmap_offer = 1; g.a.smallmap_bn = &fold; }
     GI_TRY(gemm_run(net, 1, g));
+    if (g.a.smallmap_applied) { bn_smallmap_commit(net, s, net->unorm[k]); continue; }
     if (g.a.fold_applied) { bn_acc_commit(net, s, net->unorm[k], sp); continue; }
     if (drop.p > 0.f && !sp.use) GI_TRY(dropout_draw(net, drop, opix * net->ch[k - 1]));
     if (fused && sp.use) {
diff --git a/gan-inpainting_amd/csrc/smallmap.hip b/gan-inpainting_amd/csrc/smallmap.hip
--- /dev/null
+++ b/gan-inpainting_amd/csrc/smallmap.hip
@@ -0,0 +1,336 @@
+#include "common.h"
+#include "bn_acc.h"
+#include "igemm_plan.h"
+
+namespace {
+
+struct KPS {
+  const char* in;
+  const char* w;
+  char* out;
+  int M, Hs, Ws;
+  int Hin, Win, Hout, Wout;
+  int cin, ldin, coffin;
+  int cout, ldout, coffout;
+  int Ktot;
+  int relu_cend;
+  int act_out;
+  int inpix;
+  int live;
+  int bn;
+  BnAccP fa;
+  char* fdst; int flddst, fcoffdst, fact;
+  uint8_t* fdrop; float fdrop_scale; uint64_t fdrop_seed; uint32_t fdrop_thresh;
+};
+
+__device__ __forceinline__ int sm_slot(int row, int c) { return (c ^ (row >> 1) ^ (row >> 2)) & 7; }
+
+__device__ __forceinline__ void glds16_sm(const char* src, char* lds_wave_base) {
+  __builtin_amdgcn_global_load_lds((const __attribute__((address_space(1))) void*)src, (__attribute__((address_space(3))) void*)lds_wave_base,
+                                   16, 0, 0);
+}
+
+template <int MODE, int NT>
+__global__ void __launch_bounds__(256, 1) smallmap_kernel(KPS p) {
+  constexpr int NPIECE = (MODE == 1 ? 1 : 4) * NT * 16 / 8 / 4 > 0 ? (MODE == 1 ? 1 : 4) * NT * 16 / 8 / 4 : 1;
+  constexpr int NV = MODE == 1 ? NT : (NT + 3) / 4;
+  extern __shared__ __attribute__((aligned(16))) char smem[];
+  const int tid = threadIdx.x, lane = tid & 63;
+  const int wave = __builtin_amdgcn_readfirstlane(tid >> 6);
+  const int lr = lane & 15, lq = lane >> 4;
+  const int n0 = blockIdx.x * GI_SMALLMAP_SLICE;
+  const int zrow = ((p.inpix + 7) & ~7);
+  const int buf_bytes = (zrow + 1) * 128;
+
+  int un[4] = {0, 0, 0, 0};
+  int nun = 0;
+  {
+    int idx = 0;
+#pragma unroll
+    for (int u = 0; u < 16; ++u) {
+      if ((p.live >> u) & 1) {
+        const bool mine = MODE == 1 ? (u >> 2) == wave : (idx & 3) == wave;
+        if (mine) {
+#pragma unroll
+          for (int j = 0; j < 4; ++j)
+            if (nun == j) un[j] = u;
+          ++nun;
+        }
+        ++idx;
+      }
+    }
+  }
+
+  int rbase[NT];
+  unsigned amask[NT];
+#pragma unroll
+  for (int t = 0; t < NT; ++t) {
+    rbase[t] = 0;
+    amask[t] = 0;
+    const int m = t * 16 + lr;
+    if (m < p.M) {
+      const int x = m % p.Ws, tt0 = m / p.Ws, y = tt0 % p.Hs, n = tt0 / p.Hs;
+      if (MODE == 1) {
+        const int ph = wave, y0 = y + (ph >> 1), x0 = x + (ph & 1);
+        rbase[t] = (n * p.Hs + y0) * p.Ws + x0;
+#pragma unroll
+        for (int tt = 0; tt < 4; ++tt) {
+          const int iy = y0 - (tt >> 1), ix = x0 - (tt & 1);
+          if (iy >= 0 && iy < p.Hs && ix >= 0 && ix < p.Ws) amask[t] |= 1u << tt;
+        }
+      } else {
+        const int y0 = 2 * y - 1, x0 = 2 * x - 1;
+        rbase[t] = (n * p.Hin + y0) * p.Win + x0;
+#pragma unroll
+        for (int tt = 0; tt < 16; ++tt) {
+          const int iy = y0 + (tt >> 2), ix = x0 + (tt & 3);
+          if (iy >= 0 && iy < p.Hin && ix >= 0 && ix < p.Win) amask[t] |= 1u << tt;
+        }
+      }
+    }
+  }
+
+  const char* wl = p.w + ((int64_t)(n0 + lr) * p.Ktot + lq * 8) * 2;
+  int64_t uoff[4];
+#pragma unroll
+  for (int j = 0; j < 4; ++j) {
+    const int u = un[j];
+    uoff[j] = MODE == 1 ? ((int64_t)(u >> 2) * p.cout * p.Ktot + (int64_t)(u & 3) * p.cin) * 2 : (int64_t)u * p.cin * 2;
+  }
+  u4_t wcur[4][2], wnxt[4][2];
+  auto load_w = [&](int c0, u4_t (&wf)[4][2]) {
+#pragma unroll
+    for (int j = 0; j < 4; ++j) {
+      wf[j][0] = *(const u4_t*)(wl + uoff[j] + c0 * 2);
+      wf[j][1] = *(const u4_t*)(wl + uoff[j] + c0 * 2 + 64);
+    }
+  };
+  const int npiece = (p.inpix + 7) >> 3;
+  const char* src[NPIECE];
+#pragma unroll
+  for (int it = 0; it < NPIECE; ++it) {
+    const int q = min(it * 4 + wave, npiece - 1), row = q * 8 + (lane >> 3), rowc = min(row, p.inpix - 1);
+    src[it] = p.in + ((int64_t)rowc * p.ldin + p.coffin + sm_slot(row, lane & 7) * 8) * 2;
+  }
+  auto load_in = [&](char* buf, int c0) {
+#pragma unroll
+    for (int it = 0; it < NPIECE; ++it) {
+      const int q = min(it * 4 + wave, npiece - 1);
+      glds16_sm(src[it] + c0 * 2, buf + q * 1024);
+    }
+  };
+
+  f4_t acc[NT];
+#pragma unroll
+  for (int t = 0; t < NT; ++t) acc[t] = f4_t{0.f, 0.f, 0.f, 0.f};
+
+  auto compute = [&](const char* buf, const u4_t (&wf)[4][2], short rfloor) {
+#pragma unroll
+    for (int j = 0; j < 4; ++j) {
+      if (j >= nun) break;
+      const int u = un[j];
+      const int tt = MODE == 1 ? (u & 3) : u;
+      const int toff = MODE == 1 ? -((tt >> 1) * p.Ws + (tt & 1)) : (tt >> 2) * p.Win + (tt & 3);
+      const h8_t w0 = __builtin_bit_cast(h8_t, wf[j][0]), w1 = __builtin_bit_cast(h8_t, wf[j][1]);
+      h8_t a0[NT], a1[NT];
+#pragma unroll
+      for (int t = 0; t < NT; ++t) {
+        const int row = ((amask[t] >> tt) & 1u) ? rbase[t] + toff : zrow;
+        const char* a = buf + row * 128;
+        a0[t] = *(const h8_t*)(a + (sm_slot(row, lq) << 4));
+        a1[t] = *(const h8_t*)(a + (sm_slot(row, 4 + lq) << 4));
+      }
+#pragma unroll
+      for (int t = 0; t < NT; ++t) acc[t] = __builtin_amdgcn_mfma_f32_16x16x32_f16(w0, relu7(a0[t], rfloor), acc[t], 0, 0, 0);
+#pragma unroll
+      for (int t = 0; t < NT; ++t) acc[t] = __builtin_amdgcn_mfma_f32_16x16x32_f16(w1, relu7(a1[t], rfloor), acc[t], 0, 0, 0);
+    }
+  };
+
+  if (tid < 16) *(u4_t*)(smem + (tid >> 3) * buf_bytes + zrow * 128 + (tid & 7) * 16) = u4_t{0u, 0u, 0u, 0u};
+  load_in(smem, 0);
+  load_w(0, wcur);
+  asm volatile("s_waitcnt vmcnt(0)" ::: "memory");
+  __syncthreads();
+  const int nchunk = p.cin / 64;
+  for (int c = 0; c < nchunk; ++c) {
+    const bool more = c + 1 < nchunk;
+    const int cn = more ? (c + 1) * 64 : c * 64;
+    char* cur = smem + (c & 1) * buf_bytes;
+    char* nxt = smem + ((c & 1) ^ 1) * buf_bytes;
+    load_w(cn, wnxt);
+    load_in(nxt, cn);
+    compute(cur, wcur, c * 64 < p.relu_cend ? (short)0 : (short)-32768);
+#pragma unroll
+    for (int j = 0; j < 4; ++j) { wcur[j][0] = wnxt[j][0]; wcur[j][1] = wnxt[j][1]; }
+    asm volatile("s_waitcnt vmcnt(0)" ::: "memory");
+    __syncthreads();
+  }
+
+  float* colsum = (float*)(smem + 4 * 8 * 1024);
+  float* aff = colsum + 4 * 16 * 2;
+  f4_t v[NV];
+  int opix[NV];
+  if constexpr (MODE == 1) {
+#pragma unroll
+    for (int t = 0; t < NT; ++t) {
+      v[t] = acc[t];
+      opix[t] = -1;
+      const int m = t * 16 + lr;
+      if (m < p.M) {
+        const int x = m % p.Ws, tt0 = m / p.Ws, y = tt0 % p.Hs, n = tt0 / p.Hs;
+        opix[t] = (n * p.Hout + 2 * y + (wave >> 1)) * p.Wout + 2 * x + (wave & 1);
+      }
+    }
+  } else {
+    f4_t* red = (f4_t*)smem;
+#pragma unroll
+    for (int t = 0; t < NT; ++t) red[(wave * NT + t) * 64 + lane] = acc[t];
+    __syncthreads();
+#pragma unroll
+    for (int i = 0; i < NV; ++i) {
+      const int t = wave + 4 * i;
+      v[i] = f4_t{0.f, 0.f, 0.f, 0.f};
+      opix[i] = -1;
+      if (t < NT) {
+#pragma unroll
+        for (int w = 0; w < 4; ++w) v[i] += red[(w * NT + t) * 64 + lane];
+        if (t * 16 + lr < p.M) opix[i] = t * 16 + lr;
+      }
+    }
+  }
+  const int ch = 4 * lq;
+
+  if (!p.bn) {
+    gi_with_act(p.act_out, [&](auto ACTc) {
+      constexpr int ACT = decltype(ACTc)::value;
+#pragma unroll
+      for (int i = 0; i < NV; ++i) {
+        if (opix[i] >= 0) {
+          h4_t o;
+#pragma unroll
+          for (int r = 0; r < 4; ++r) o[r] = (half_t)gi_act_c<ACT>(v[i][r]);
+          *(h4_t*)(p.out + ((int64_t)opix[i] * p.ldout + p.coffout + n0 + ch) * 2) = o;
+        }
+      }
+    });
+    return;
+  }
+
+  {
+    float s[4], q[4];
+#pragma unroll
+    for (int r = 0; r < 4; ++r) {
+      s[r] = 0.f;
+      q[r] = 0.f;
+#pragma unroll
+      for (int i = 0; i < NV; ++i) { s[r] += v[i][r]; q[r] += v[i][r] * v[i][r]; }
+      s[r] = gi_row16_sum(s[r]);
+      q[r] = gi_row16_sum(q[r]);
+    }
+    if (lr == 0) {
+#pragma unroll
+      for (int r = 0; r < 4; ++r) { colsum[(wave * 16 + ch + r) * 2] = s[r]; colsum[(wave * 16 + ch + r) * 2 + 1] = q[r]; }
+    }
+  }
+  __syncthreads();
+  if (tid < 16) {
+    const int c = n0 + tid;
+    const float gam = p.fa.gamma[c], bet = p.fa.beta[c], rm = p.fa.rmean[c], rv = p.fa.rvar[c];
+    float s = 0.f, q = 0.f;
+#pragma unroll
+    for (int w = 0; w < 4; ++w) { s += colsum[(w * 16 + tid) * 2]; q += colsum[(w * 16 + tid) * 2 + 1]; }
+    float sc, sh;
+    bn_from_totals(p.fa, c, 0, true, (double)s, (double)q, gam, bet, rm, rv, sc, sh);
+    aff[tid] = sc;
+    aff[16 + tid] = sh;
+  }
+  __syncthreads();
+  float fsc[4], fsh[4];
+#pragma unroll
+  for (int r = 0; r < 4; ++r) { fsc[r] = aff[ch + r]; fsh[r] = aff[16 + ch + r]; }
+  gi_with_act(p.fact, [&](auto ACTc) {
+    constexpr int ACT = decltype(ACTc)::value;
+#pragma unroll
+    for (int i = 0; i < NV; ++i) {
+      if (opix[i] < 0) continue;
+      h4_t raw;
+#pragma unroll
+      for (int r = 0; r < 4; ++r) raw[r] = (half_t)v[i][r];
+      *(h4_t*)(p.out + ((int64_t)opix[i] * p.ldout + p.coffout + n0 + ch) * 2) = raw;
+      float o[4];
+#pragma unroll
+      for (int r = 0; r < 4; ++r) o[r] = gi_act_c<ACT>(fmaf((float)raw[r], fsc[r], fsh[r]));
+      if (p.fdrop) {
+        const int64_t e0 = (int64_t)opix[i] * p.cout + n0 + ch;
+        unsigned keep;
+        if (p.fdrop_thresh) {
+          keep = 0;
+#pragma unroll
+          for (int r = 0; r < 4; ++r) keep |= (unsigned)dropout_keep(p.fdrop_seed, e0 + r, p.fdrop_thresh) << (8 * r);
+          *(unsigned*)(p.fdrop + e0) = keep;
+        } else keep = *(const unsigned*)(p.fdrop + e0);
+#pragma unroll
+        for (int r = 0; r < 4; ++r) o[r] = ((keep >> (8 * r)) & 0xFFu) ? o[r] * p.fdrop_scale : 0.f;
+      }
+      h4_t o4;
+#pragma unroll
+      for (int r = 0; r < 4; ++r) o4[r] = (half_t)o[r];
+      *(h4_t*)(p.fdst + ((int64_t)opix[i] * p.flddst + p.fcoffdst + n0 + ch) * 2) = o4;
+    }
+  });
+}
+
+int live_units(int mode, int Hs, int Ws) {
+  int live = 0;
+  for (int u = 0; u < 16; ++u) {
+    bool any = false;
+    for (int y = 0; y < Hs && !any; ++y)
+      for (int x = 0; x < Ws && !any; ++x) {
+        int iy, ix, H, W;
+        if (mode == 1) { const int ph = u >> 2, tt = u & 3; iy = y + (ph >> 1) - (tt >> 1); ix = x + (ph & 1) - (tt & 1); H = Hs; W = Ws; }
+        else { iy = 2 * y - 1 + (u >> 2); ix = 2 * x - 1 + (u & 3); H = 2 * Hs; W = 2 * Ws; }
+        any = iy >= 0 && iy < H && ix >= 0 && ix < W;
+      }
+    if (any) live |= 1 << u;
+  }
+  return live;
+}
+
+}
+
+int launch_smallmap(hipStream_t st, const IgemmPlan& p, const IgemmArgs& a) {
+  const int mode = p.mode;
+  KPS kp;
+  kp.in = (const char*)a.in; kp.w = (const char*)a.w; kp.out = (char*)a.out;
+  kp.M = a.n * a.Hs * a.Ws; kp.Hs = a.Hs; kp.Ws = a.Ws;
+  if (mode == 1) { kp.Hin = a.Hs; kp.Win = a.Ws; kp.Hout = 2 * a.Hs; kp.Wout = 2 * a.Ws; }
+  else { kp.Hin = 2 * a.Hs; kp.Win = 2 * a.Ws; kp.Hout = a.Hs; kp.Wout = a.Ws; }
+  kp.cin = a.cin; kp.ldin = a.ldin; kp.coffin = a.coffin;
+  kp.cout = a.cout; kp.ldout = a.ldout; kp.coffout = a.coffout;
+  kp.Ktot = (mode == 1 ? 4 : 16) * a.cin;
+  kp.relu_cend = a.relu_in ? (a.relu_cend > 0 ? a.relu_cend : a.cin) : 0;
+  kp.act_out = a.act_out;
+  kp.inpix = kp.M * (mode == 0 ? 4 : 1);
+  kp.live = live_units(mode, a.Hs, a.Ws);
+  const int tiles = (kp.M + 15) / 16;
+  GI_REQUIRE(tiles * 16 <= GI_SMALLMAP_MAXPIX && 2 * (((kp.inpix + 7) & ~7) + 1) * 128 <= p.lds_bytes, "smallmap: internal: the plan took a layer of %d pixels", kp.M);
+  kp.bn = p.smallmap_bn ? 1 : 0;
+  if (p.smallmap_bn) {
+    const IgemmFold& f = *a.smallmap_bn;
+    gi_fill_acc_params(kp.fa, f.bn);
+    kp.fa.acc = nullptr; kp.fa.zero_next = nullptr; kp.fa.zero_words = 0;
+    kp.fdst = (char*)f.dst; kp.flddst = f.lddst; kp.fcoffdst = f.coffdst; kp.fact = f.act;
+    kp.fdrop = f.drop_mask; kp.fdrop_scale = f.drop_scale; kp.fdrop_seed = f.drop_seed;
+    kp.fdrop_thresh = f.drop_p > 0.f ? gi_dropout_thresh(f.drop_p) : 0u;
+  } else {
+    kp.fa = BnAccP{}; kp.fdst = nullptr; kp.flddst = kp.fcoffdst = kp.fact = 0;
+    kp.fdrop = nullptr; kp.fdrop_scale = 1.f; kp.fdrop_seed = 0; kp.fdrop_thresh = 0;
+  }
+#define GI_KSM(V, MODE_, NAME) \
+  case V: return tiles <= 2 ? gi_launch_lds<smallmap_kernel<MODE_, 2>>(dim3(p.grid), 256, p.lds_bytes, p.lds_attr_bytes, st, kp) \
+                            : gi_launch_lds<smallmap_kernel<MODE_, 8>>(dim3(p.grid), 256, p.lds_bytes, p.lds_attr_bytes, st, kp);
+  switch (p.variant & 1) { GI_SMALLMAP_KERNELS(GI_KSM) }
+#undef GI_KSM
+  return GI_ERR_INVALID;
+}
diff --git a/include/ganinpaint.h b/include/ganinpaint.h
--- a/include/ganinpaint.h
+++ b/include/ganinpaint.h
@@ -29,6 +29,7 @@
 int gi_get_option(const char* name, int* value);
 const char* gi_debug_last_kernel(void);
 int gi_debug_fold_count(void);
+int gi_debug_smallmap_count(int with_bn);
 
 int gi_ctx_create(int device_id, void* hip_stream, gi_ctx** out);
 int gi_ctx_destroy(gi_ctx* ctx);
@@ -319,6 +320,10 @@
   unsigned long long* zero_next; int zero_words;
 } gi_bn_acc_args;
 int gi_debug_bn_finalize_acc(gi_ctx* ctx, int c, const gi_bn_acc_args* b);
+int gi_debug_smallmap_forward(gi_ctx* ctx, int mode, const void* in, const void* w, void* out, int n, int Hs, int Ws, int cin, int ldin,
+                              int cout, int ldout, int coffout, int relu_in, int relu_cend, int act_out, const gi_bn_acc_args* bn,
+                              void* dst, int lddst, int coffdst, int act, uint8_t* drop_mask, float drop_scale, uint64_t drop_seed,
+                              float drop_p);
 int gi_debug_bn_apply_acc(gi_ctx* ctx, int dtype, const void* x, void* y, int64_t pixels, int c, int ldy, int coffy, int act,
                           uint8_t* drop_mask, float drop_scale, uint64_t drop_seed, float drop_p, const gi_bn_acc_args* b,
                           const void* side_src, void* side_dst, int64_t side_bytes);
```
